# junshutang/Make-It-3D

Hardware: AMD Instinct MI355X
Metric: SDS train-steps/sec (NeRF render+SD U-Net fwd+bwd) @128x128 (higher is better)
Workload: dtype f32 hash grid (fp32 gather, fp32 gradient contributions accumulated in 64-bit fixed point) + f16 MFMA MLP (torch.autocast semantics; the planes between gather, MLP and scatter hold the binary16 values autocast rounds them to), f16 U-Net

## Files before the change

### include/mi3d.h

```cpp
#ifndef MI3D_H
#define MI3D_H

#include <stddef.h>
#include <stdint.h>

#ifdef __cplusplus
extern "C" {
#endif

#define MI3D_MAX_LEVELS 16
#define MI3D_MAX_POINTS 16

int mi3d_abi_version(void);
const char *mi3d_last_error_string(int err);


int mi3d_near_far_from_aabb(const float *rays_o, const float *rays_d, const float *aabb, uint32_t N,
                            float min_near, float *nears, float *fars, void *stream);
int mi3d_sph_from_ray(const float *rays_o, const float *rays_d, float radius, uint32_t N, float *coords,
                      void *stream);
int mi3d_morton3D(const int32_t *coords, uint32_t N, int32_t *indices, void *stream);
int mi3d_morton3D_invert(const int32_t *indices, uint32_t N, int32_t *coords, void *stream);
int mi3d_packbits(const float *grid, uint32_t N, float density_thresh, uint8_t *bitfield, void *stream);

int mi3d_march_rays_train(const float *rays_o, const float *rays_d, const uint8_t *grid, float bound,
                          float dt_gamma, uint32_t max_steps, uint32_t N, uint32_t C, uint32_t H, uint32_t M,
                          const float *nears, const float *fars, float *xyzs, float *dirs, float *deltas,
                          int32_t *rays, int32_t *counter, const float *noises, void *stream);
int mi3d_march_zero_tail(const int32_t *counter, uint32_t align, uint32_t M, float *xyzs, float *dirs,
                         float *deltas, void *stream);

int mi3d_composite_rays_train_forward(const float *sigmas, const float *rgbs, const float *deltas,
                                      const int32_t *rays, uint32_t M, uint32_t N, float T_thresh,
                                      float *weights_sum, float *depth, float *image, void *stream);
int mi3d_composite_rays_train_backward(const float *grad_weights_sum, const float *grad_image,
                                       const float *sigmas, const float *rgbs, const float *deltas,
                                       const int32_t *rays, const float *weights_sum, const float *image,
                                       uint32_t M, uint32_t N, float T_thresh, float *grad_sigmas,
                                       float *grad_rgbs, void *stream);
int mi3d_composite_rays_train_backward_depth(const float *grad_weights_sum, const float *grad_depth,
                                             const float *grad_image, const float *sigmas, const float *rgbs,
                                             const float *deltas, const int32_t *rays, const float *weights_sum,
                                             const float *depth, const float *image, uint32_t M, uint32_t N,
                                             float T_thresh, float *grad_sigmas, float *grad_rgbs, void *stream);
int mi3d_composite_sdf_rays_train_forward(const float *sigmas, const float *rgbs, const float *deltas,
                                          const int32_t *rays, uint32_t M, uint32_t N, float T_thresh,
                                          float *weights_sum, float *depth, float *image, void *stream);
int mi3d_composite_sdf_rays_train_backward(const float *grad_weights_sum, const float *grad_image,
                                           const float *sigmas, const float *rgbs, const float *deltas,
                                           const int32_t *rays, const float *weights_sum, const float *image,
                                           uint32_t M, uint32_t N, float T_thresh, float *grad_sigmas,
                                           float *grad_rgbs, void *stream);

int mi3d_march_rays(uint32_t n_alive, uint32_t n_step, const int32_t *rays_alive, const float *rays_t,
                    const float *rays_o, const float *rays_d, float bound, float dt_gamma, uint32_t max_steps,
                    uint32_t C, uint32_t H, const uint8_t *grid, const float *nears, const float *fars,
                    float *xyzs, float *dirs, float *deltas, const float *noises, void *stream);
int mi3d_composite_rays(uint32_t n_alive, uint32_t n_step, float T_thresh, int32_t *rays_alive, float *rays_t,
                        const float *sigmas, const float *rgbs, const float *normals, const float *deltas,
                        float *weights_sum, float *depth, float *image, float *normal, void *stream);
int mi3d_composite_sdf_rays(uint32_t n_alive, uint32_t n_step, float T_thresh, int32_t *rays_alive,
                            float *rays_t, const float *sigmas, const float *rgbs, const float *deltas,
                            float *weights_sum, float *depth, float *image, void *stream);

int mi3d_infer_begin(int32_t *ctl, int32_t *rays_alive, uint32_t N, uint32_t align, void *stream);
int mi3d_march_rays_ctl(const int32_t *ctl, uint32_t n_alive_max, const int32_t *rays_alive, const float *rays_t,
                        const float *rays_o, const float *rays_d, float bound, float dt_gamma, uint32_t max_steps,
                        uint32_t C, uint32_t H, const uint8_t *grid, const float *fars, float *xyzs, float *dirs,
                        float *deltas, const float *noises, void *stream);
int mi3d_composite_rays_ctl(const int32_t *ctl, uint32_t n_alive_max, float T_thresh, int32_t *rays_alive,
                            float *rays_t, const float *sigmas, const float *rgbs, const float *normals,
                            const float *deltas, float *weights_sum, float *depth, float *image, float *normal,
                            void *stream);
int mi3d_compact_alive_ctl(int32_t *ctl, const int32_t *rays_alive_in, int32_t *rays_alive_out, uint32_t N,
                           uint32_t align, uint32_t max_steps, void *stream);

int mi3d_infer_begin2(int32_t *ctl, int32_t *rays_alive, uint32_t N, uint32_t budget_rows, uint32_t step_min,
                      uint32_t step_max, void *stream);
int mi3d_march_rays_compact_ctl(int32_t *ctl, uint32_t n_alive_max, const int32_t *rays_alive, const float *rays_t,
                                const float *rays_o, const float *rays_d, float bound, float dt_gamma, uint32_t max_steps,
                                uint32_t C, uint32_t H, const uint8_t *grid, const float *fars, uint32_t rows_cap,
                                float *xyzs, float *dirs, float *deltas, int32_t *ray_slab, float *t_next,
                                const float *noises, void *stream);
int mi3d_composite_rays_compact_ctl(const int32_t *ctl, uint32_t n_alive_max, float T_thresh, int32_t *rays_alive,
                                    float *rays_t, const int32_t *ray_slab, const float *t_next, const float *sigmas,
                                    const float *rgbs, const float *normals, const float *deltas, float *weights_sum,
                                    float *depth, float *image, float *normal, void *stream);
int mi3d_compact_alive_ctl2(int32_t *ctl, const int32_t *rays_alive_in, int32_t *rays_alive_out, uint32_t N,
                            uint32_t max_steps, void *stream);


uint32_t mi3d_hashgrid_levels(uint32_t n_levels, uint32_t base_resolution, float per_level_scale,
                              uint32_t log2_hashmap_size, uint32_t *offsets_host, uint32_t *resolutions_host,
                              float *scales_host);

int mi3d_hashgrid_forward(const float *x, uint32_t n, const float *params, uint32_t n_levels,
                          uint32_t base_resolution, float per_level_scale, uint32_t log2_hashmap_size,
                          float *out, void *stream);
int mi3d_hashgrid_backward(const float *x, uint32_t n, const float *dout, uint32_t n_levels,
                           uint32_t base_resolution, float per_level_scale, uint32_t log2_hashmap_size,
                           float *grad_params, void *stream);


int mi3d_grid_encode_points(const float *x, const float *x2, uint32_t n, const int32_t *count,
                            const float *offsets_host, uint32_t P0, uint32_t P, float bound, const float *params,
                            uint32_t n_levels, uint32_t base_resolution, float per_level_scale,
                            uint32_t log2_hashmap_size, float *out, void *stream);
int mi3d_grid_encode_points_planes(const float *x, const float *x2, uint32_t n, const float *offsets_host, uint32_t P0,
                                   uint32_t P, float bound, const float *params, uint32_t n_levels,
                                   uint32_t base_resolution, float per_level_scale, uint32_t log2_hashmap_size, float step,
                                   void *out_planes, int out_half, void *stream);
int mi3d_grid_encode_points_planes_counted(const float *x, const float *x2, uint32_t n, const int32_t *count,
                                           const float *offsets_host, uint32_t P0, uint32_t P, float bound,
                                           const float *params, uint32_t n_levels, uint32_t base_resolution,
                                           float per_level_scale, uint32_t log2_hashmap_size, float step, void *out_planes,
                                           int out_half, void *stream);
int mi3d_grid_scatter_points(const float *x, const float *x2, uint32_t n, const int32_t *count,
                             const float *offsets_host, uint32_t P0, uint32_t P, float bound, const float *dout,
                             uint32_t n_levels, uint32_t base_resolution, float per_level_scale,
                             uint32_t log2_hashmap_size, float step, float *grad_params, void *stream);

size_t mi3d_grid_scatter_binned_workspace(uint32_t n, uint32_t P, float bound, float step, uint32_t n_levels,
                                          uint32_t base_resolution, float per_level_scale, uint32_t log2_hashmap_size);
int mi3d_grid_scatter_binned(const float *x, const float *x2, uint32_t n, const float *offsets_host, uint32_t P0,
                             uint32_t P, float bound, const void *dout_planes, int dout_half, uint32_t n_levels,
                             uint32_t base_resolution, float per_level_scale, uint32_t log2_hashmap_size, float step,
                             void *workspace, size_t workspace_bytes, float *grad_params, void *stream);
int mi3d_grid_scatter_binned_plus(const float *x, const float *x2, uint32_t n, const float *offsets_host, uint32_t P0,
                                  uint32_t P, float bound, const void *dout_planes, const void *extra_point0_planes,
                                  int dout_half, uint32_t n_levels, uint32_t base_resolution, float per_level_scale,
                                  uint32_t log2_hashmap_size, float step, void *workspace, size_t workspace_bytes,
                                  float *grad_params, void *stream);

int mi3d_grid_encode_plan(uint32_t n, float bound, float step, uint32_t n_levels, uint32_t base_resolution,
                          float per_level_scale, uint32_t log2_hashmap_size, uint32_t *n_segments, uint32_t *segments);
int mi3d_grid_scatter_plan(uint32_t n, uint32_t P, float bound, float step, uint32_t n_levels, uint32_t base_resolution,
                           float per_level_scale, uint32_t log2_hashmap_size, size_t workspace_bytes,
                           unsigned long long *out);
int mi3d_grid_level_routes(uint32_t n_levels, uint32_t base_resolution, float per_level_scale, uint32_t log2_hashmap_size,
                           int stencil_points, int32_t *kinds);


int mi3d_mlp_supported(uint32_t dim_in, uint32_t dim_hidden, uint32_t dim_out, uint32_t num_layers);
int mi3d_mlp_forward(const void *x, uint32_t x_plane_rows, int planes_half, uint32_t n, const float *W1,
                     const float *b1, const float *W2, const float *b2,
                     const float *W3, const float *b3, uint32_t dim_in, uint32_t dim_hidden, uint32_t dim_out,
                     int half_mode, float *out, void *stream);
int mi3d_mlp_forward_counted(const void *x, uint32_t x_plane_rows, int planes_half, uint32_t n, const int32_t *count,
                             uint32_t n_stride, const float *W1, const float *b1, const float *W2, const float *b2,
                             const float *W3, const float *b3, uint32_t dim_in, uint32_t dim_hidden, uint32_t dim_out,
                             int half_mode, float *out, void *stream);
int mi3d_mlp_backward(const void *x, uint32_t x_plane_rows, int planes_half, const float *dout, uint32_t n,
                      const float *W1, const float *b1, const float *W2, const float *b2, const float *W3,
                      const float *b3, uint32_t dim_in, uint32_t dim_hidden, uint32_t dim_out, int half_mode, void *dx,
                      uint32_t dx_plane_rows, float *dW1, float *db1, float *dW2, float *db2, float *dW3, float *db3,
                      void *stream);


int mi3d_field_head_forward(const float *h, const float *x, const float *x2, uint32_t n, const float *offsets_host,
                            uint32_t P, float bound, float blob_density, float blob_radius, float epsilon, float *sigma,
                            float *albedo, float *normal, float *normal2, void *stream);
int mi3d_field_head_forward_counted(const float *h, const float *x, const float *x2, uint32_t n, const int32_t *count,
                                    const float *offsets_host, uint32_t P, float bound, float blob_density,
                                    float blob_radius, float epsilon, float *sigma, float *albedo, float *normal,
                                    float *normal2, void *stream);
int mi3d_field_head_backward(const float *h, const float *x, const float *x2, uint32_t n, const float *offsets_host,
                             uint32_t P, uint32_t P_active, float bound, float blob_density, float blob_radius,
                             float epsilon, const float *dsigma, const float *dalbedo, const float *dnormal,
                             const float *dnormal2, float *dh, void *stream);


int mi3d_sumsq_accumulate(const float *x, size_t n, float *acc, void *stream);
int mi3d_adan_step(float *param, float *grad, float *exp_avg, float *exp_avg_sq, float *exp_avg_diff,
                   float *neg_pre_grad, size_t count, const float *grad_sumsq, float max_grad_norm, float clip_eps,
                   int first_step, float beta1, float beta2, float beta3, float bias_correction1,
                   float bias_correction2, float bias_correction3_sqrt, float lr, float weight_decay, float eps,
                   int no_prox, void *stream);


size_t mi3d_points_rasterize_workspace(uint32_t P, uint32_t H, uint32_t W, float radius);
int mi3d_points_rasterize(const float *points_ndc, uint32_t P, uint32_t H, uint32_t W, float radius,
                          uint32_t points_per_pixel, void *workspace, size_t workspace_bytes, int32_t *idx, float *zbuf,
                          float *dists, void *stream);
int mi3d_points_composite_forward(const int32_t *idx, const float *dists, uint32_t H, uint32_t W, uint32_t points_per_pixel,
                                  const float *features, uint32_t C, double radius, float *out, void *stream);
int mi3d_points_composite_backward(const int32_t *idx, const float *dists, uint32_t H, uint32_t W,
                                   uint32_t points_per_pixel, const float *grad_out, uint32_t C, double radius,
                                   float *grad_features, void *stream);


size_t mi3d_mc_workspace(uint32_t Rx, uint32_t Ry, uint32_t Rz);
int mi3d_mc_case(uint32_t case_index, int8_t *edges_host);
int mi3d_mc_count(const float *vol, uint32_t Rx, uint32_t Ry, uint32_t Rz, float iso, void *ws, size_t ws_bytes,
                  unsigned long long *counts, void *stream);
int mi3d_mc_scan(uint32_t Rx, uint32_t Ry, uint32_t Rz, void *ws, size_t ws_bytes, unsigned long long *counts,
                 void *stream);
int mi3d_mc_emit(const float *vol, uint32_t Rx, uint32_t Ry, uint32_t Rz, float iso, const float *origin_host,
                 const float *spacing_host, void *ws, size_t ws_bytes, unsigned long long *counts, float *vertices,
                 unsigned long long nv_cap, int32_t *triangles, unsigned long long nt_cap, void *stream);


uint32_t mi3d_atlas_cell(unsigned long long nt, uint32_t T);
int mi3d_atlas_uv(unsigned long long nt, uint32_t T, float *vt, void *stream);
int mi3d_atlas_positions(const float *vertices, unsigned long long nv, const int32_t *triangles, unsigned long long nt,
                         uint32_t T, uint32_t ssaa, uint32_t row0, uint32_t rows, float *xyz, int32_t *owner,
                         unsigned long long *bad, void *stream);
int mi3d_texture_pack(const float *albedo, const int32_t *owner, uint32_t T, uint32_t ssaa, uint32_t rows, uint8_t *image,
                      void *stream);


uint32_t mi3d_groupnorm_chunks(uint32_t HW);
int mi3d_groupnorm_stats(const void *x, uint32_t B, uint32_t C, uint32_t HW, uint32_t G, float *ws, void *stream);
int mi3d_groupnorm_act_forward(const void *x, const float *ws, const float *weight, const float *bias, uint32_t B,
                               uint32_t C, uint32_t HW, uint32_t G, float eps, int act, void *y, float *mean, float *rstd,
                               void *stream);
int mi3d_groupnorm_act_backward_sums(const void *x, const void *dy, const float *mean, const float *rstd,
                                     const float *weight, const float *bias, uint32_t B, uint32_t C, uint32_t HW,
                                     uint32_t G, int act, float *partial, void *stream);
int mi3d_groupnorm_act_backward(const void *x, const void *dy, const float *mean, const float *rstd, const float *weight,
                                const float *bias, const float *partial, uint32_t B, uint32_t C, uint32_t HW, uint32_t G,
                                int act, void *dx, void *stream);


int mi3d_canny_classify(const uint8_t *image, uint32_t H, uint32_t W, int32_t low, int32_t high, uint8_t *cls,
                        unsigned long long *counts, void *stream);
int mi3d_canny_hysteresis(uint8_t *cls, uint32_t H, uint32_t W, uint32_t sweeps, int32_t *changed, void *stream);


size_t mi3d_pc_unproject_workspace(uint32_t H, uint32_t W);
int mi3d_pc_unproject(const double *depth, const uint8_t *mask, uint32_t H, uint32_t W, const double *kinv_host,
                      const double *c2w_host, void *ws, size_t ws_bytes, double *points, unsigned long long cap,
                      unsigned long long *count, void *stream);
int mi3d_pc_project(const double *points, unsigned long long n, const double *rt_host, const double *k_host, double *xy,
                    double *z, void *stream);
int mi3d_pc_zmin(const double *points, unsigned long long n, const double *rt_host, const double *k_host, uint32_t H,
                 uint32_t W, unsigned long long *zkeys, void *stream);
int mi3d_pc_visible(const double *points, unsigned long long n, const double *rt_host, const double *k_host, uint32_t H,
                    uint32_t W, const unsigned long long *zkeys, uint8_t *visible, void *stream);
int mi3d_box_morph(const float *src, float *dst, uint32_t H, uint32_t W, uint32_t kh, uint32_t kw, int dilate,
                   void *stream);
int mi3d_pc_cano_filter(const double *points, unsigned long long n, const double *rt_host, const double *k_host,
                        const float *cano_depth, uint32_t H, uint32_t W, uint8_t *keep, void *stream);
int mi3d_pc_colour(const double *points, unsigned long long n, const double *rt_host, const double *k_host,
                   const float *image, uint32_t H, uint32_t W, float *colour, void *stream);

#ifdef __cplusplus
}
#endif
#endif
```

### make-it-3d_amd/csrc/field.hip

```cpp
#include <hip/hip_runtime.h>

#include "../../include/mi3d.h"
#include "mi3d_dev.h"
#include "lds_transpose.h"

#ifndef MI3D_MLP_LDS_TRANSPOSE
#define MI3D_MLP_LDS_TRANSPOSE 1
#endif

namespace {

constexpr int kWave = 64;
constexpr int kWavesPerWG = 4;
constexpr int DIN = 32, HID = 64, DOUT = 4;
constexpr int NTH = HID / 32;

using f32x16 = __attribute__((ext_vector_type(16))) float;
using f32x4 = __attribute__((ext_vector_type(4))) float;
using f32x2 = __attribute__((ext_vector_type(2))) float;
using half8 = __attribute__((ext_vector_type(8))) _Float16;
using half2v = __attribute__((ext_vector_type(2))) _Float16;
using ushort8v = __attribute__((ext_vector_type(8))) unsigned short;

inline hipStream_t as_stream(void *s) { return reinterpret_cast<hipStream_t>(s); }

__device__ __forceinline__ int rowmap(int q, int h) { return (q & 3) + 8 * (q >> 2) + 4 * h; }

struct F16 {
    using elem = _Float16;
    static constexpr int kUnits = 2;
    static constexpr bool kLdsTranspose = MI3D_MLP_LDS_TRANSPOSE != 0;
    struct KB { half8 v[2]; };
    __device__ static __forceinline__ float round(float x) { return (float)(_Float16)x; }
    __device__ static __forceinline__ void set(KB &k, int q, float x) { k.v[q >> 3][q & 7] = (_Float16)x; }
    __device__ static __forceinline__ void set_pair_bits(KB &k, int j, uint32_t bits) {
        const half2v hv = __builtin_bit_cast(half2v, bits);
        k.v[j >> 2][2 * (j & 3)] = hv[0];
        k.v[j >> 2][2 * (j & 3) + 1] = hv[1];
    }
    __device__ static __forceinline__ void mma(f32x16 &acc, const KB &a, const KB &b) {
        acc = __builtin_amdgcn_mfma_f32_32x32x16_f16(a.v[0], b.v[0], acc, 0, 0, 0);
        acc = __builtin_amdgcn_mfma_f32_32x32x16_f16(a.v[1], b.v[1], acc, 0, 0, 0);
    }
    [[maybe_unused]] static constexpr int kSteps = 2;
    __device__ static __forceinline__ void mma_step(f32x16 &acc, const KB &a, const KB &b, int s) {
        acc = __builtin_amdgcn_mfma_f32_32x32x16_f16(a.v[s], b.v[s], acc, 0, 0, 0);
    }
    __device__ static __forceinline__ void mma_lo(f32x16 &acc, const KB &a, const KB &b) {
        acc = __builtin_amdgcn_mfma_f32_32x32x16_f16(a.v[0], b.v[0], acc, 0, 0, 0);
    }
    __device__ static __forceinline__ KB load_block(const char *blk, int lane) {
        KB k;
        k.v[0] = *reinterpret_cast<const half8 *>(blk + (0 * kWave + lane) * 16);
        k.v[1] = *reinterpret_cast<const half8 *>(blk + (1 * kWave + lane) * 16);
        return k;
    }
    __device__ static __forceinline__ KB relu(const f32x16 &acc) {
        KB k;
#pragma unroll
        for (int j = 0; j < 8; ++j) {
            const f32x2 pr = {acc[2 * j], acc[2 * j + 1]};
            half2v hv = __builtin_convertvector(pr, half2v);
            hv = __builtin_elementwise_maximum(hv, half2v{(_Float16)0, (_Float16)0});
            k.v[j >> 2][2 * (j & 3)] = hv[0];
            k.v[j >> 2][2 * (j & 3) + 1] = hv[1];
        }
        return k;
    }
    __device__ static __forceinline__ KB masked(const f32x16 &d, const KB &act) {
        KB k;
        const unsigned ones = 0x00010001u;
        using u32x4 = __attribute__((ext_vector_type(4))) uint32_t;
#pragma unroll
        for (int u = 0; u < 2; ++u) {
            const u32x4 aw = __builtin_bit_cast(u32x4, act.v[u]);
            u32x4 o;
#pragma unroll
            for (int j = 0; j < 4; ++j) {
                const f32x2 pr = {d[8 * u + 2 * j], d[8 * u + 2 * j + 1]};
                const unsigned dv = __builtin_bit_cast(unsigned, __builtin_convertvector(pr, half2v));
                unsigned m = aw[j];
                asm("v_pk_min_u16 %0, %1, %2\n\tv_pk_mul_lo_u16 %0, %0, %3"
                    : "=&v"(m) : "v"(m), "s"(ones), "v"(dv));
                o[j] = m;
            }
            k.v[u] = __builtin_bit_cast(half8, o);
        }
        return k;
    }
    __device__ static __forceinline__ KB cast(const f32x16 &acc) {
        KB k;
#pragma unroll
        for (int j = 0; j < 8; ++j) {
            const f32x2 pr = {acc[2 * j], acc[2 * j + 1]};
            const half2v hv = __builtin_convertvector(pr, half2v);
            k.v[j >> 2][2 * (j & 3)] = hv[0];
            k.v[j >> 2][2 * (j & 3) + 1] = hv[1];
        }
        return k;
    }
    __device__ static __forceinline__ float sum(const KB &k) {
        float s = 0.f;
        const half2v ones = {(_Float16)1, (_Float16)1};
        using u32x4 = __attribute__((ext_vector_type(4))) uint32_t;
#pragma unroll
        for (int u = 0; u < 2; ++u) {
            const u32x4 w = __builtin_bit_cast(u32x4, k.v[u]);
#pragma unroll
            for (int j = 0; j < 4; ++j) {
                const uint32_t wj = w[j];
                s = __builtin_amdgcn_fdot2(__builtin_bit_cast(half2v, wj), ones, s, false);
            }
        }
        return s;
    }
};

struct F32 {
    using elem = float;
    static constexpr int kUnits = 4;
    static constexpr bool kLdsTranspose = false;
    struct KB { float v[16]; };
    __device__ static __forceinline__ float round(float x) { return x; }
    __device__ static __forceinline__ void set(KB &k, int q, float x) { k.v[q] = x; }
    __device__ static __forceinline__ void set_pair_bits(KB &k, int j, uint32_t bits) {
        const half2v hv = __builtin_bit_cast(half2v, bits);
        k.v[2 * j] = (float)hv[0];
        k.v[2 * j + 1] = (float)hv[1];
    }
    __device__ static __forceinline__ void mma(f32x16 &acc, const KB &a, const KB &b) {
#pragma unroll
        for (int q = 0; q < 16; ++q) acc = __builtin_amdgcn_mfma_f32_32x32x2f32(a.v[q], b.v[q], acc, 0, 0, 0);
    }
    static constexpr int kSteps = 16;
    __device__ static __forceinline__ void mma_step(f32x16 &acc, const KB &a, const KB &b, int s) {
        acc = __builtin_amdgcn_mfma_f32_32x32x2f32(a.v[s], b.v[s], acc, 0, 0, 0);
    }
    __device__ static __forceinline__ void mma_lo(f32x16 &acc, const KB &a, const KB &b) {
#pragma unroll
        for (int q = 0; q < 8; ++q) acc = __builtin_amdgcn_mfma_f32_32x32x2f32(a.v[q], b.v[q], acc, 0, 0, 0);
    }
    __device__ static __forceinline__ KB load_block(const char *blk, int lane) {
        KB k;
#pragma unroll
        for (int u = 0; u < 4; ++u) {
            const f32x4 t = *reinterpret_cast<const f32x4 *>(blk + (u * kWave + lane) * 16);
            k.v[4 * u] = t[0]; k.v[4 * u + 1] = t[1]; k.v[4 * u + 2] = t[2]; k.v[4 * u + 3] = t[3];
        }
        return k;
    }
    __device__ static __forceinline__ KB relu(const f32x16 &acc) {
        KB k;
#pragma unroll
        for (int q = 0; q < 16; ++q) k.v[q] = fmaxf(acc[q], 0.f);
        return k;
    }
    __device__ static __forceinline__ KB masked(const f32x16 &d, const KB &act) {
        KB k;
#pragma unroll
        for (int q = 0; q < 16; ++q) k.v[q] = act.v[q] > 0.f ? d[q] : 0.f;
        return k;
    }
    __device__ static __forceinline__ KB cast(const f32x16 &acc) {
        KB k;
#pragma unroll
        for (int q = 0; q < 16; ++q) k.v[q] = acc[q];
        return k;
    }
    __device__ static __forceinline__ float sum(const KB &k) {
        float s = 0.f;
#pragma unroll
        for (int q = 0; q < 16; ++q) s += k.v[q];
        return s;
    }
};

template <class P> constexpr int block_bytes() { return P::kUnits * kWave * 16; }

enum : int {
    B_W1 = 0,
    B_W2 = B_W1 + NTH,
    B_W3 = B_W2 + NTH * NTH,
    B_W3T = B_W3 + NTH,
    B_W2T = B_W3T + NTH,
    B_W1T = B_W2T + NTH * NTH,
    B_ID = B_W1T + NTH,
    B_ALL_COUNT = B_ID + 1,
};

struct Weights {
    const float *W1, *b1, *W2, *b2, *W3, *b3;
};

template <class P>
__device__ void build_blocks(char *lds, float *bias , const Weights &w, int n_blocks) {
    using T = typename P::elem;
    for (int e = threadIdx.x; e < n_blocks * kWave * 16; e += blockDim.x) {
        const int blk = e / (kWave * 16), r = e % (kWave * 16), lane = r / 16, q = r % 16;
        const int nl = lane & 31, h = lane >> 5;
        const int kd = rowmap(q, h), kx = 16 * h + q;
        float v = 0.f;
        if (blk < B_W2) {
            const int tn = blk - B_W1;
            v = w.W1[(32 * tn + nl) * DIN + kx];
        } else if (blk < B_W3) {
            const int tn = (blk - B_W2) / NTH, tk = (blk - B_W2) % NTH;
            v = w.W2[(32 * tn + nl) * HID + 32 * tk + kd];
        } else if (blk < B_W3T) {
            const int tk = blk - B_W3;
            v = nl < DOUT ? w.W3[nl * HID + 32 * tk + kd] : 0.f;
        } else if (blk < B_W2T) {
            const int tn = blk - B_W3T;
            v = kx < DOUT ? w.W3[kx * HID + 32 * tn + nl] : 0.f;
        } else if (blk < B_W1T) {
            const int tn = (blk - B_W2T) / NTH, tk = (blk - B_W2T) % NTH;
            v = w.W2[(32 * tk + kd) * HID + 32 * tn + nl];
        } else if (blk < B_ID) {
            const int tk = blk - B_W1T;
            v = w.W1[(32 * tk + kd) * DIN + nl];
        } else {
            v = nl == kx ? 1.f : 0.f;
        }
        constexpr int per_unit = 16 / (int)sizeof(T);
        T *dst = reinterpret_cast<T *>(lds + (size_t)blk * block_bytes<P>() + ((q / per_unit) * kWave + lane) * 16);
        dst[q % per_unit] = (T)v;
    }
    for (int e = threadIdx.x; e < HID + HID + 32; e += blockDim.x) {
        float v = 0.f;
        if (e < HID) v = w.b1[e];
        else if (e < 2 * HID) v = w.b2[e - HID];
        else if (e - 2 * HID < DOUT) v = w.b3[e - 2 * HID];
        bias[e] = P::round(v);
    }
}

__device__ __forceinline__ void load_rows_raw(const float *__restrict__ x, size_t row, size_t n, int h,
                                              size_t plane_rows, float (&raw)[16], int planes_half = 0) {
    row = row < n ? row : n - 1;
    if (plane_rows != 0 && planes_half) {
#pragma unroll
        for (int j = 0; j < 8; ++j) {
            const uint32_t u = reinterpret_cast<const uint32_t *>(x)[(size_t)(8 * h + j) * plane_rows + row];
            raw[2 * j] = (float)__builtin_bit_cast(_Float16, (unsigned short)(u & 0xFFFFu));
            raw[2 * j + 1] = (float)__builtin_bit_cast(_Float16, (unsigned short)(u >> 16));
        }
    } else if (plane_rows == 0) {
        const f32x4 *src = reinterpret_cast<const f32x4 *>(x + row * DIN + 16 * h);
#pragma unroll
        for (int c = 0; c < 4; ++c) {
            const f32x4 t = src[c];
#pragma unroll
            for (int i = 0; i < 4; ++i) raw[4 * c + i] = t[i];
        }
    } else {
#pragma unroll
        for (int j = 0; j < 8; ++j) {
            const f32x2 t = *reinterpret_cast<const f32x2 *>(x + ((size_t)(8 * h + j) * plane_rows + row) * 2);
            raw[2 * j] = t[0];
            raw[2 * j + 1] = t[1];
        }
    }
}
template <class P> __device__ __forceinline__ typename P::KB rows_kb(const float (&raw)[16]) {
    typename P::KB k;
#pragma unroll
    for (int q = 0; q < 16; ++q) P::set(k, q, raw[q]);
    return k;
}
[[maybe_unused]] __device__ __forceinline__ void load_rows_half(const float *__restrict__ x, size_t row, size_t n, int h,
                                               size_t plane_rows, uint32_t (&u)[8]) {
    row = row < n ? row : n - 1;
#pragma unroll
    for (int j = 0; j < 8; ++j) u[j] = reinterpret_cast<const uint32_t *>(x)[(size_t)(8 * h + j) * plane_rows + row];
}
template <class P> __device__ __forceinline__ typename P::KB rows_kb_half(const uint32_t (&u)[8]) {
    typename P::KB k;
#pragma unroll
    for (int j = 0; j < 8; ++j) P::set_pair_bits(k, j, u[j]);
    return k;
}

__device__ __forceinline__ f32x4 load_dout_raw(const float *__restrict__ dout, size_t row, size_t n) {
    return *reinterpret_cast<const f32x4 *>(dout + (row < n ? row : n - 1) * DOUT);
}
template <class P> __device__ __forceinline__ typename P::KB dout_kb(const f32x4 &t, bool keep) {
    typename P::KB k;
#pragma unroll
    for (int q = 0; q < 16; ++q) P::set(k, q, (q < 4 && keep) ? t[q] : 0.f);
    return k;
}

__device__ __forceinline__ f32x16 splat(float v) {
    f32x16 a;
#pragma unroll
    for (int q = 0; q < 16; ++q) a[q] = v;
    return a;
}
__device__ __forceinline__ f32x16 bias_rows(const float *bias, int h) {
    f32x16 a;
#pragma unroll
    for (int q = 0; q < 16; ++q) a[q] = bias[rowmap(q, h)];
    return a;
}
struct Grads {
    float *dW1, *db1, *dW2, *db2, *dW3, *db3;
};

template <class P, int U, int WPS, bool HP>
__global__ __launch_bounds__(kWave *kWavesPerWG, WPS) void k_mlp_backward(const float *x, uint32_t x_planes,
                                                                           int , const float *__restrict__ dout,
                                                                           uint32_t n, Weights w, float *dx,
                                                                           uint32_t dx_planes, Grads g) {
    extern __shared__ __attribute__((aligned(16))) char lds[];
    float *bias = reinterpret_cast<float *>(lds + (size_t)B_ALL_COUNT * block_bytes<P>());
    build_blocks<P>(lds, bias, w, B_ALL_COUNT);
    __syncthreads();
    const int lane = threadIdx.x & (kWave - 1), p = lane & 31, h = lane >> 5;
    const uint32_t wave = blockIdx.x * kWavesPerWG + threadIdx.x / kWave, n_waves = gridDim.x * kWavesPerWG;
    const uint32_t n_tiles = (n + 31) / 32;
    using KB = typename P::KB;
    auto blk = [&](int b) {
        int l = lane;
        asm volatile("" : "+v"(l));
        return P::load_block(lds + (size_t)b * block_bytes<P>(), l);
    };

    f32x16 gW2[NTH][NTH], gW1[NTH], gW3[NTH];
    float gb1[NTH], gb2[NTH], gb3 = 0.f;
#pragma unroll
    for (int a = 0; a < NTH; ++a) {
        gW1[a] = splat(0.f); gW3[a] = splat(0.f); gb1[a] = 0.f; gb2[a] = 0.f;
#pragma unroll
        for (int b = 0; b < NTH; ++b) gW2[a][b] = splat(0.f);
    }

    float raw[HP ? 1 : U][16];
    uint32_t rawh[HP ? U : 1][8];
    f32x4 dor[U];
#pragma unroll
    for (int u = 0; u < U; ++u) {
        const size_t r0 = ((size_t)wave + (size_t)u * n_waves) * 32 + p;
        if constexpr (HP) load_rows_half(x, r0, n, h, x_planes, rawh[u]);
        else load_rows_raw(x, r0, n, h, x_planes, raw[u]);
        dor[u] = load_dout_raw(dout, r0, n);
    }
    for (uint32_t tile = wave; tile < n_tiles; tile += U * n_waves) {
        size_t row[U];
        bool valid[U];
        KB X[U], dO[U];
#pragma unroll
        for (int u = 0; u < U; ++u) {
            row[u] = ((size_t)tile + (size_t)u * n_waves) * 32 + p;
            valid[u] = row[u] < n;
            if constexpr (HP) X[u] = rows_kb_half<P>(rawh[u]);
            else X[u] = rows_kb<P>(raw[u]);
            dO[u] = dout_kb<P>(dor[u], valid[u] && h == 0);
        }
        if (tile + U * n_waves < n_tiles) {
#pragma unroll
            for (int u = 0; u < U; ++u) {
                const size_t rn = ((size_t)tile + (size_t)(U + u) * n_waves) * 32 + p;
                if constexpr (HP) load_rows_half(x, rn, n, h, x_planes, rawh[u]);
                else load_rows_raw(x, rn, n, h, x_planes, raw[u]);
                dor[u] = load_dout_raw(dout, rn, n);
            }
        }

        KB H1[U][NTH], H2[U][NTH], dH2[U][NTH], dH1[U][NTH];
        {
            f32x16 acc[U][NTH];
#pragma unroll
            for (int t = 0; t < NTH; ++t)
#pragma unroll
                for (int u = 0; u < U; ++u) acc[u][t] = bias_rows(bias + 32 * t, h);
            {
                KB Wb[NTH];
#pragma unroll
                for (int t = 0; t < NTH; ++t) Wb[t] = blk(B_W1 + t);
#pragma unroll
                for (int st = 0; st < P::kSteps; ++st)
#pragma unroll
                    for (int t = 0; t < NTH; ++t)
#pragma unroll
                        for (int u = 0; u < U; ++u) P::mma_step(acc[u][t], Wb[t], X[u], st);
            }
#pragma unroll
            for (int t = 0; t < NTH; ++t)
#pragma unroll
                for (int u = 0; u < U; ++u) H1[u][t] = P::relu(acc[u][t]);
        }
        {
            f32x16 acc[U][NTH];
#pragma unroll
            for (int t = 0; t < NTH; ++t)
#pragma unroll
                for (int u = 0; u < U; ++u) acc[u][t] = bias_rows(bias + HID + 32 * t, h);
#pragma unroll
            for (int tk = 0; tk < NTH; ++tk) {
                KB Wb[NTH];
#pragma unroll
                for (int t = 0; t < NTH; ++t) Wb[t] = blk(B_W2 + t * NTH + tk);
#pragma unroll
                for (int st = 0; st < P::kSteps; ++st)
#pragma unroll
                    for (int t = 0; t < NTH; ++t)
#pragma unroll
                        for (int u = 0; u < U; ++u) P::mma_step(acc[u][t], Wb[t], H1[u][tk], st);
            }
#pragma unroll
            for (int t = 0; t < NTH; ++t)
#pragma unroll
                for (int u = 0; u < U; ++u) H2[u][t] = P::relu(acc[u][t]);
        }
        {
            f32x16 acc[U][NTH];
            KB Wb[NTH];
#pragma unroll
            for (int t = 0; t < NTH; ++t) Wb[t] = blk(B_W3T + t);
#pragma unroll
            for (int t = 0; t < NTH; ++t)
#pragma unroll
                for (int u = 0; u < U; ++u) { acc[u][t] = splat(0.f); P::mma_lo(acc[u][t], Wb[t], dO[u]); }
#pragma unroll
            for (int t = 0; t < NTH; ++t)
#pragma unroll
                for (int u = 0; u < U; ++u) dH2[u][t] = P::masked(acc[u][t], H2[u][t]);
        }
        {
            f32x16 acc[U][NTH];
#pragma unroll
            for (int t = 0; t < NTH; ++t)
#pragma unroll
                for (int u = 0; u < U; ++u) acc[u][t] = splat(0.f);
#pragma unroll
            for (int tk = 0; tk < NTH; ++tk) {
                KB Wb[NTH];
#pragma unroll
                for (int t = 0; t < NTH; ++t) Wb[t] = blk(B_W2T + t * NTH + tk);
#pragma unroll
                for (int st = 0; st < P::kSteps; ++st)
#pragma unroll
                    for (int t = 0; t < NTH; ++t)
#pragma unroll
                        for (int u = 0; u < U; ++u) P::mma_step(acc[u][t], Wb[t], dH2[u][tk], st);
            }
#pragma unroll
            for (int t = 0; t < NTH; ++t)
#pragma unroll
                for (int u = 0; u < U; ++u) dH1[u][t] = P::masked(acc[u][t], H1[u][t]);
        }
        {
            f32x16 acc[U];
#pragma unroll
            for (int u = 0; u < U; ++u) acc[u] = splat(0.f);
#pragma unroll
            for (int tk = 0; tk < NTH; ++tk) {
                const KB Wb = blk(B_W1T + tk);
#pragma unroll
                for (int st = 0; st < P::kSteps; ++st)
#pragma unroll
                    for (int u = 0; u < U; ++u) P::mma_step(acc[u], Wb, dH1[u][tk], st);
            }
#pragma unroll
            for (int u = 0; u < U; ++u) {
                if (valid[u] && !dx_planes) {
                    float *dst = dx + row[u] * DIN + 4 * h;
#pragma unroll
                    for (int c = 0; c < 4; ++c) {
                        f32x4 o = {acc[u][4 * c], acc[u][4 * c + 1], acc[u][4 * c + 2], acc[u][4 * c + 3]};
                        __builtin_nontemporal_store(o, reinterpret_cast<f32x4 *>(dst + 8 * c));
                    }
                } else if (valid[u] && HP) {
#pragma unroll
                    for (int c = 0; c < 4; ++c) {
                        const size_t lvl = 4 * c + 2 * h;
                        const half2v a = __builtin_convertvector((f32x2){acc[u][4 * c], acc[u][4 * c + 1]}, half2v);
                        const half2v b = __builtin_convertvector((f32x2){acc[u][4 * c + 2], acc[u][4 * c + 3]}, half2v);
                        reinterpret_cast<uint32_t *>(dx)[lvl * dx_planes + row[u]] = __builtin_bit_cast(uint32_t, a);
                        reinterpret_cast<uint32_t *>(dx)[(lvl + 1) * dx_planes + row[u]] = __builtin_bit_cast(uint32_t, b);
                    }
                } else if (valid[u]) {
#pragma unroll
                    for (int c = 0; c < 4; ++c) {
                        f32x2 a = {acc[u][4 * c], acc[u][4 * c + 1]}, b = {acc[u][4 * c + 2], acc[u][4 * c + 3]};
                        const size_t lvl = 4 * c + 2 * h;
                        __builtin_nontemporal_store(a, reinterpret_cast<f32x2 *>(dx + (lvl * dx_planes + row[u]) * 2));
                        __builtin_nontemporal_store(b, reinterpret_cast<f32x2 *>(dx + ((lvl + 1) * dx_planes + row[u]) * 2));
                    }
                }
            }
        }

        KB H1p[U][NTH];
        {
            f32x16 acc[U][NTH];
#pragma unroll
            for (int t = 0; t < NTH; ++t)
#pragma unroll
                for (int u = 0; u < U; ++u) acc[u][t] = splat(bias[32 * t + p]);
            KB Wb[NTH];
#pragma unroll
            for (int t = 0; t < NTH; ++t) Wb[t] = blk(B_W1 + t);
#pragma unroll
            for (int st = 0; st < P::kSteps; ++st)
#pragma unroll
                for (int t = 0; t < NTH; ++t)
#pragma unroll
                    for (int u = 0; u < U; ++u) P::mma_step(acc[u][t], X[u], Wb[t], st);
#pragma unroll
            for (int t = 0; t < NTH; ++t)
#pragma unroll
                for (int u = 0; u < U; ++u) H1p[u][t] = P::relu(acc[u][t]);
        }
        KB dH2p[U][NTH];
        {
            KB H2p[U][NTH], dOp[U];
            {
                f32x16 acc[U][NTH];
#pragma unroll
                for (int t = 0; t < NTH; ++t)
#pragma unroll
                    for (int u = 0; u < U; ++u) acc[u][t] = splat(bias[HID + 32 * t + p]);
#pragma unroll
                for (int tk = 0; tk < NTH; ++tk) {
                    KB Wb[NTH];
#pragma unroll
                    for (int t = 0; t < NTH; ++t) Wb[t] = blk(B_W2 + t * NTH + tk);
#pragma unroll
                    for (int st = 0; st < P::kSteps; ++st)
#pragma unroll
                        for (int t = 0; t < NTH; ++t)
#pragma unroll
                            for (int u = 0; u < U; ++u) P::mma_step(acc[u][t], H1[u][tk], Wb[t], st);
                }
#pragma unroll
                for (int t = 0; t < NTH; ++t)
#pragma unroll
                    for (int u = 0; u < U; ++u) H2p[u][t] = P::relu(acc[u][t]);
            }
            {
                const KB Id = blk(B_ID);
                f32x16 tO[U];
#pragma unroll
                for (int u = 0; u < U; ++u) { tO[u] = splat(0.f); P::mma_lo(tO[u], dO[u], Id); }
#pragma unroll
                for (int u = 0; u < U; ++u) { dOp[u] = P::cast(tO[u]); gb3 += P::sum(dOp[u]); }
            }
#pragma unroll
            for (int u = 0; u < U; ++u)
#pragma unroll
                for (int st = 0; st < P::kSteps; ++st)
#pragma unroll
                    for (int t = 0; t < NTH; ++t) P::mma_step(gW3[t], dOp[u], H2p[u][t], st);
            {
                f32x16 d[U][NTH];
                KB Wb[NTH];
#pragma unroll
                for (int t = 0; t < NTH; ++t) Wb[t] = blk(B_W3T + t);
#pragma unroll
                for (int t = 0; t < NTH; ++t)
#pragma unroll
                    for (int u = 0; u < U; ++u) { d[u][t] = splat(0.f); P::mma_lo(d[u][t], dO[u], Wb[t]); }
#pragma unroll
                for (int t = 0; t < NTH; ++t)
#pragma unroll
                    for (int u = 0; u < U; ++u) {
                        dH2p[u][t] = P::masked(d[u][t], H2p[u][t]);
                        gb2[t] += P::sum(dH2p[u][t]);
                    }
            }
        }
#pragma unroll
        for (int u = 0; u < U; ++u)
#pragma unroll
            for (int st = 0; st < P::kSteps; ++st)
#pragma unroll
                for (int ti = 0; ti < NTH; ++ti)
#pragma unroll
                    for (int tj = 0; tj < NTH; ++tj) P::mma_step(gW2[ti][tj], dH2p[u][ti], H1p[u][tj], st);
        {
            KB dH1p[U][NTH], Xp[U];
            {
                f32x16 d[U][NTH];
#pragma unroll
                for (int t = 0; t < NTH; ++t)
#pragma unroll
                    for (int u = 0; u < U; ++u) d[u][t] = splat(0.f);
#pragma unroll
                for (int tk = 0; tk < NTH; ++tk) {
                    KB Wb[NTH];
#pragma unroll
                    for (int t = 0; t < NTH; ++t) Wb[t] = blk(B_W2T + t * NTH + tk);
#pragma unroll
                    for (int st = 0; st < P::kSteps; ++st)
#pragma unroll
                        for (int t = 0; t < NTH; ++t)
#pragma unroll
                            for (int u = 0; u < U; ++u) P::mma_step(d[u][t], dH2[u][tk], Wb[t], st);
                }
#pragma unroll
                for (int t = 0; t < NTH; ++t)
#pragma unroll
                    for (int u = 0; u < U; ++u) {
                        dH1p[u][t] = P::masked(d[u][t], H1p[u][t]);
                        gb1[t] += P::sum(dH1p[u][t]);
                    }
            }
            {
                const KB Id = blk(B_ID);
                f32x16 tX[U];
#pragma unroll
                for (int u = 0; u < U; ++u) tX[u] = splat(0.f);
#pragma unroll
                for (int st = 0; st < P::kSteps; ++st)
#pragma unroll
                    for (int u = 0; u < U; ++u) P::mma_step(tX[u], X[u], Id, st);
#pragma unroll
                for (int u = 0; u < U; ++u) Xp[u] = P::cast(tX[u]);
            }
#pragma unroll
            for (int u = 0; u < U; ++u)
#pragma unroll
                for (int st = 0; st < P::kSteps; ++st)
#pragma unroll
                    for (int t = 0; t < NTH; ++t) P::mma_step(gW1[t], dH1p[u][t], Xp[u], st);
        }
    }

    __syncthreads();
    float *red = reinterpret_cast<float *>(lds);
    constexpr int OFF_W1 = 0, OFF_B1 = OFF_W1 + HID * DIN, OFF_W2 = OFF_B1 + HID, OFF_B2 = OFF_W2 + HID * HID,
                  OFF_W3 = OFF_B2 + HID, OFF_B3 = OFF_W3 + DOUT * HID, TOTAL = OFF_B3 + DOUT;
    for (int e = threadIdx.x; e < TOTAL; e += blockDim.x) red[e] = 0.f;
    __syncthreads();
#pragma unroll
    for (int q = 0; q < 16; ++q) {
        const int r = rowmap(q, h);
#pragma unroll
        for (int ti = 0; ti < NTH; ++ti) {
            atomicAdd(&red[OFF_W1 + (32 * ti + r) * DIN + p], gW1[ti][q]);
#pragma unroll
            for (int tj = 0; tj < NTH; ++tj) atomicAdd(&red[OFF_W2 + (32 * ti + r) * HID + 32 * tj + p], gW2[ti][tj][q]);
            if (r < DOUT) atomicAdd(&red[OFF_W3 + r * HID + 32 * ti + p], gW3[ti][q]);
        }
    }
#pragma unroll
    for (int t = 0; t < NTH; ++t) {
        atomicAdd(&red[OFF_B1 + 32 * t + p], gb1[t]);
        atomicAdd(&red[OFF_B2 + 32 * t + p], gb2[t]);
    }
    if (p < DOUT) atomicAdd(&red[OFF_B3 + p], gb3);
    __syncthreads();
    for (int e = threadIdx.x; e < TOTAL; e += blockDim.x) {
        const float v = red[e];
        float *dst = e < OFF_B1 ? g.dW1 + (e - OFF_W1)
                   : e < OFF_W2 ? g.db1 + (e - OFF_B1)
                   : e < OFF_B2 ? g.dW2 + (e - OFF_W2)
                   : e < OFF_W3 ? g.db2 + (e - OFF_B2)
                   : e < OFF_B3 ? g.dW3 + (e - OFF_W3)
                                : g.db3 + (e - OFF_B3);
        if (v != 0.f) unsafeAtomicAdd(dst, v);
    }
}

template <int NTH, int LAYERS> struct Blk {
    static constexpr int W1 = 0;
    static constexpr int W2 = W1 + NTH;
    static constexpr int W3 = W2 + (LAYERS == 3 ? NTH * NTH : 0);
    static constexpr int FWD_COUNT = W3 + NTH;
    static constexpr int W3T = FWD_COUNT;
    static constexpr int W2T = W3T + NTH;
    static constexpr int W1T = W2T + (LAYERS == 3 ? NTH * NTH : 0);
    static constexpr int IDX = W1T + NTH;
    static constexpr int IDD = IDX + 1;
    static constexpr int ALL_COUNT = IDD + 1;
    static constexpr int BIAS_TILES = 2 * NTH + 1;
};

template <class P, int NTH, int LAYERS>
__device__ void build_blocks_g(char *lds, float *biasT, const Weights &w, int din, int n_blocks) {
    using T = typename P::elem;
    using B = Blk<NTH, LAYERS>;
    constexpr int H = 32 * NTH;
    for (int e = threadIdx.x; e < n_blocks * kWave * 16; e += blockDim.x) {
        const int blk = e / (kWave * 16), r = e % (kWave * 16), lane = r / 16, q = r % 16;
        const int nl = lane & 31, h = lane >> 5;
        const int kd = rowmap(q, h), kx = 16 * h + q;
        float v = 0.f;
        if (blk < B::W2) {
            const int tn = blk - B::W1;
            v = kx < din ? w.W1[(32 * tn + nl) * din + kx] : 0.f;
        } else if (blk < B::W3) {
            const int tn = (blk - B::W2) / NTH, tk = (blk - B::W2) % NTH;
            v = w.W2[(32 * tn + nl) * H + 32 * tk + kd];
        } else if (blk < B::W3T) {
            const int tk = blk - B::W3;
            v = nl < DOUT ? w.W3[nl * H + 32 * tk + kd] : 0.f;
        } else if (blk < B::W2T) {
            const int tn = blk - B::W3T;
            v = kx < DOUT ? w.W3[kx * H + 32 * tn + nl] : 0.f;
        } else if (blk < B::W1T) {
            const int tn = (blk - B::W2T) / NTH, tk = (blk - B::W2T) % NTH;
            v = w.W2[(32 * tk + kd) * H + 32 * tn + nl];
        } else if (blk < B::IDX) {
            const int tk = blk - B::W1T;
            v = nl < din ? w.W1[(32 * tk + kd) * din + nl] : 0.f;
        } else if (blk == B::IDX) {
            v = nl == kx ? 1.f : 0.f;
        } else {
            v = nl == kd ? 1.f : 0.f;
        }
        constexpr int per_unit = 16 / (int)sizeof(T);
        T *dst = reinterpret_cast<T *>(lds + (size_t)blk * block_bytes<P>() + ((q / per_unit) * kWave + lane) * 16);
        dst[q % per_unit] = (T)v;
    }
    for (int e = threadIdx.x; e < B::BIAS_TILES * 32; e += blockDim.x) {
        const int tile = e / 32, h = (e % 32) / 16, q = e % 16, row = rowmap(q, h);
        float v = 0.f;
        if (tile < NTH) v = w.b1[32 * tile + row];
        else if (tile < 2 * NTH) v = LAYERS == 3 ? w.b2[32 * (tile - NTH) + row] : 0.f;
        else v = row < DOUT ? w.b3[row] : 0.f;
        biasT[e] = P::round(v);
    }
}
__device__ __forceinline__ f32x16 bias_tile(const float *biasT, int tile, int h) {
    const f32x4 *src = reinterpret_cast<const f32x4 *>(biasT + (tile * 2 + h) * 16);
    f32x16 a;
#pragma unroll
    for (int c = 0; c < 4; ++c) {
        const f32x4 t = src[c];
        a[4 * c] = t[0]; a[4 * c + 1] = t[1]; a[4 * c + 2] = t[2]; a[4 * c + 3] = t[3];
    }
    return a;
}

template <bool FULL = false>
__device__ __forceinline__ void load_rows_half_g(const float *__restrict__ x, size_t row, size_t n, int h,
                                                 size_t plane_rows, uint32_t last_plane, uint32_t (&u)[8]) {
    row = row < n ? row : n - 1;
    if constexpr (FULL) {
        const uint32_t *src = reinterpret_cast<const uint32_t *>(x) + ((size_t)(8 * h) * plane_rows + row);
#pragma unroll
        for (int j = 0; j < 8; ++j) u[j] = src[(size_t)j * plane_rows];
        return;
    }
#pragma unroll
    for (int j = 0; j < 8; ++j) {
        const uint32_t pl = (uint32_t)(8 * h + j) < last_plane ? (uint32_t)(8 * h + j) : last_plane;
        u[j] = reinterpret_cast<const uint32_t *>(x)[(size_t)pl * plane_rows + row];
    }
}
__device__ __forceinline__ void load_rows_raw_g(const float *__restrict__ x, size_t row, size_t n, int h,
                                                size_t plane_rows, uint32_t din, float (&raw)[16]) {
    row = row < n ? row : n - 1;
    const uint32_t last_plane = din / 2 - 1;
    if (plane_rows == 0 && din == DIN) {
        const f32x4 *src = reinterpret_cast<const f32x4 *>(x + row * DIN + 16 * h);
#pragma unroll
        for (int c = 0; c < 4; ++c) {
            const f32x4 t = src[c];
#pragma unroll
            for (int i = 0; i < 4; ++i) raw[4 * c + i] = t[i];
        }
    } else if (plane_rows == 0) {
#pragma unroll
        for (int q = 0; q < 16; ++q) {
            const uint32_t f = (uint32_t)(16 * h + q) < din ? (uint32_t)(16 * h + q) : din - 1;
            raw[q] = x[row * din + f];
        }
    } else {
#pragma unroll
        for (int j = 0; j < 8; ++j) {
            const uint32_t pl = (uint32_t)(8 * h + j) < last_plane ? (uint32_t)(8 * h + j) : last_plane;
            const f32x2 t = *reinterpret_cast<const f32x2 *>(x + ((size_t)pl * plane_rows + row) * 2);
            raw[2 * j] = t[0];
            raw[2 * j + 1] = t[1];
        }
    }
}

template <class P, int NTH, int LAYERS, bool HP>
__global__ __launch_bounds__(kWave *kWavesPerWG, 2) void k_mlp_fwd_g(const float *__restrict__ x, uint32_t x_planes,
                                                                        uint32_t n, uint32_t din, Weights w,
                                                                        float *__restrict__ out,
                                                                        const int32_t *__restrict__ count, uint32_t n_stride) {
    using B = Blk<NTH, LAYERS>;
    using KB = typename P::KB;
    extern __shared__ __attribute__((aligned(16))) char lds[];
    float *biasT = reinterpret_cast<float *>(lds + (size_t)B::FWD_COUNT * block_bytes<P>());
    build_blocks_g<P, NTH, LAYERS>(lds, biasT, w, (int)din, B::FWD_COUNT);
    __syncthreads();
    const int lane = threadIdx.x & (kWave - 1), p = lane & 31, h = lane >> 5;
    const uint32_t wave = blockIdx.x * kWavesPerWG + threadIdx.x / kWave, n_waves = gridDim.x * kWavesPerWG;
    const uint32_t n_tiles = (n + 31) / 32;
    auto blk = [&](int b) {
        int l = lane;
        asm volatile("" : "+v"(l));
        return P::load_block(lds + (size_t)b * block_bytes<P>(), l);
    };
    auto bias = [&](int tile) {
        int hh = h;
        asm volatile("" : "+v"(hh));
        return bias_tile(biasT, tile, hh);
    };
    const uint32_t last_plane = din / 2 - 1;
    const uint32_t c_rows = count ? (uint32_t)max(*count, 0) : 0xFFFFFFFFu;
    for (uint32_t tile = wave; tile < n_tiles; tile += n_waves) {
        bool live = true;
        if (count) {
            const uint32_t s0 = (tile * 32u) % n_stride;
            if (s0 >= c_rows && s0 + 32u <= n_stride) continue;
            live = (s0 + (uint32_t)p) % n_stride < c_rows;
        }
        const size_t row = (size_t)tile * 32 + p;
        KB X;
        if constexpr (HP) {
            uint32_t u[8];
            load_rows_half_g(x, row, n, h, x_planes, last_plane, u);
            X = rows_kb_half<P>(u);
        } else {
            float raw[16];
            load_rows_raw_g(x, row, n, h, x_planes, din, raw);
            X = rows_kb<P>(raw);
        }
        KB H1[NTH], HL[NTH];
#pragma unroll
        for (int t = 0; t < NTH; ++t) {
            f32x16 acc = bias(t);
            P::mma(acc, blk(B::W1 + t), X);
            H1[t] = P::relu(acc);
        }
        if constexpr (LAYERS == 3) {
#pragma unroll
            for (int t = 0; t < NTH; ++t) {
                f32x16 acc = bias(NTH + t);
#pragma unroll
                for (int tk = 0; tk < NTH; ++tk) P::mma(acc, blk(B::W2 + t * NTH + tk), H1[tk]);
                HL[t] = P::relu(acc);
            }
        } else {
#pragma unroll
            for (int t = 0; t < NTH; ++t) HL[t] = H1[t];
        }
        f32x16 acc = bias(2 * NTH);
#pragma unroll
        for (int tk = 0; tk < NTH; ++tk) P::mma(acc, blk(B::W3 + tk), HL[tk]);
        if (row < n && h == 0 && live) {
            f32x4 o = {P::round(acc[0]), P::round(acc[1]), P::round(acc[2]), P::round(acc[3])};
            __builtin_nontemporal_store(o, reinterpret_cast<f32x4 *>(out + row * DOUT));
        }
    }
}

template <class P, int NTH, int LAYERS, bool HP, bool FULL>
__global__ __launch_bounds__(kWave *kWavesPerWG, 2) void k_mlp_bwd_g(const float *x, uint32_t x_planes,
                                                                        const float *__restrict__ dout, uint32_t n,
                                                                        uint32_t din, Weights w, float *dx,
                                                                        uint32_t dx_planes, Grads g) {
    using B = Blk<NTH, LAYERS>;
    using KB = typename P::KB;
    constexpr int H = 32 * NTH;
    extern __shared__ __attribute__((aligned(16))) char lds[];
    float *biasT = reinterpret_cast<float *>(lds + (size_t)B::ALL_COUNT * block_bytes<P>());
    build_blocks_g<P, NTH, LAYERS>(lds, biasT, w, (int)din, B::ALL_COUNT);
    __syncthreads();
    const int lane = threadIdx.x & (kWave - 1), p = lane & 31, h = lane >> 5;
    const uint32_t wave = blockIdx.x * kWavesPerWG + threadIdx.x / kWave, n_waves = gridDim.x * kWavesPerWG;
    const uint32_t n_tiles = (n + 31) / 32;
    int lt = lane, ht = h;
    auto blk = [&](int b) { return P::load_block(lds + (size_t)b * block_bytes<P>(), lt); };
    auto blk_fresh = [&](int b) {
        int l = lane;
        asm volatile("" : "+v"(l));
        return P::load_block(lds + (size_t)b * block_bytes<P>(), l);
    };
    auto bias = [&](int tile) { return bias_tile(biasT, tile, ht); };
    [[maybe_unused]] mi3d_tr::lds_ptr tr_wr_d = nullptr, tr_wr_x = nullptr, tr_rd = nullptr;
    if constexpr (P::kLdsTranspose) {
        mi3d_tr::lds_ptr tile = mi3d_tr::to_lds(biasT + B::BIAS_TILES * 32) + (threadIdx.x / kWave) * mi3d_tr::kTileBytes;
        tr_wr_d = tile + mi3d_tr::write_offset_d(lane);
        tr_wr_x = tile + mi3d_tr::write_offset_x(lane);
        tr_rd = tile + mi3d_tr::read_offset(lane);
    }
    auto transpose = [&](const KB &a, int id_block) {
        if constexpr (P::kLdsTranspose) {
            KB r;
            if (id_block == B::IDX) mi3d_tr::write_tile<true>(tr_wr_x, a.v[0], a.v[1]);
            else mi3d_tr::write_tile<false>(tr_wr_d, a.v[0], a.v[1]);
            mi3d_tr::read_tile(tr_rd, r.v[0], r.v[1]);
            return r;
        } else {
            f32x16 t = splat(0.f);
            P::mma(t, a, blk_fresh(id_block));
            return P::cast(t);
        }
    };
    const uint32_t last_plane = FULL ? (uint32_t)(DIN / 2 - 1) : din / 2 - 1;

    f32x16 gW1[NTH], gW2[NTH][NTH], gW3[NTH];
    float gb1[NTH], gb2[NTH], gb3 = 0.f;
#pragma unroll
    for (int a = 0; a < NTH; ++a) {
        gW1[a] = splat(0.f); gW3[a] = splat(0.f); gb1[a] = 0.f; gb2[a] = 0.f;
#pragma unroll
        for (int b = 0; b < NTH; ++b) gW2[a][b] = splat(0.f);
    }

    float raw[HP ? 1 : 16];
    uint32_t rawh[HP ? 8 : 1];
    f32x4 dor;
    {
        const size_t r0 = (size_t)wave * 32 + p;
        if constexpr (HP) load_rows_half_g<FULL && P::kLdsTranspose>(x, r0, n, h, x_planes, last_plane, rawh);
        else load_rows_raw_g(x, r0, n, h, x_planes, din, raw);
        dor = load_dout_raw(dout, r0, n);
    }
    for (uint32_t tile = wave; tile < n_tiles; tile += n_waves) {
        const size_t row = (size_t)tile * 32 + p;
        const bool valid = row < n;
        uint32_t xp = x_planes, dxp = dx_planes;
        asm volatile("" : "+s"(xp), "+s"(dxp), "+v"(lt), "+v"(ht));
        KB X;
        if constexpr (HP) X = rows_kb_half<P>(rawh);
        else X = rows_kb<P>(raw);
        const KB dO = dout_kb<P>(dor, valid && h == 0);
        auto prefetch = [&]() {
            if (tile + n_waves < n_tiles) {
                const size_t rn = ((size_t)tile + n_waves) * 32 + p;
                if constexpr (HP) load_rows_half_g<FULL && P::kLdsTranspose>(x, rn, n, P::kLdsTranspose ? ht : h, xp, last_plane, rawh);
                else load_rows_raw_g(x, rn, n, P::kLdsTranspose ? ht : h, xp, din, raw);
                dor = load_dout_raw(dout, rn, n);
            }
        };
        constexpr bool late_prefetch = P::kLdsTranspose && HP;
        if constexpr (!late_prefetch) prefetch();
        KB H1p[NTH], HL[NTH];
        {
            KB H1[NTH];
#pragma unroll
            for (int t = 0; t < NTH; ++t) {
                f32x16 acc = bias(t);
                P::mma(acc, blk(B::W1 + t), X);
                H1[t] = P::relu(acc);
            }
            if constexpr (LAYERS == 3) {
#pragma unroll
                for (int t = 0; t < NTH; ++t) {
                    f32x16 acc = bias(NTH + t);
#pragma unroll
                    for (int tk = 0; tk < NTH; ++tk) P::mma(acc, blk(B::W2 + t * NTH + tk), H1[tk]);
                    HL[t] = P::relu(acc);
                }
            } else {
#pragma unroll
                for (int t = 0; t < NTH; ++t) HL[t] = H1[t];
            }
#pragma unroll
            for (int t = 0; t < NTH; ++t) H1p[t] = transpose(H1[t], B::IDD);
        }
        KB dHL[NTH];
#pragma unroll
        for (int t = 0; t < NTH; ++t) {
            f32x16 acc = splat(0.f);
            P::mma_lo(acc, blk(B::W3T + t), dO);
            dHL[t] = P::masked(acc, HL[t]);
        }
        {
            KB dOp;
            if constexpr (P::kLdsTranspose) {
                dOp = transpose(dO, B::IDX);
            } else {
                f32x16 tO = splat(0.f);
                P::mma_lo(tO, dO, blk_fresh(B::IDX));
                dOp = P::cast(tO);
            }
            gb3 += P::sum(dOp);
#pragma unroll
            for (int t = 0; t < NTH; ++t) {
                const KB HLp = LAYERS == 3 ? transpose(HL[t], B::IDD) : H1p[t];
                P::mma(gW3[t], dOp, HLp);
            }
        }
        KB dH1p[NTH];
        if constexpr (LAYERS == 3) {
#pragma unroll
            for (int ti = 0; ti < NTH; ++ti) {
                const KB dHLp = transpose(dHL[ti], B::IDD);
                gb2[ti] += P::sum(dHLp);
#pragma unroll
                for (int tj = 0; tj < NTH; ++tj) P::mma(gW2[ti][tj], dHLp, H1p[tj]);
            }
#pragma unroll
            for (int t = 0; t < NTH; ++t) {
                f32x16 acc = splat(0.f);
#pragma unroll
                for (int tk = 0; tk < NTH; ++tk) P::mma(acc, dHL[tk], blk(B::W2T + t * NTH + tk));
                dH1p[t] = P::masked(acc, H1p[t]);
            }
        } else {
#pragma unroll
            for (int t = 0; t < NTH; ++t) dH1p[t] = transpose(dHL[t], B::IDD);
        }
        {
            const KB Xp = transpose(X, B::IDX);
            if constexpr (late_prefetch) prefetch();
#pragma unroll
            for (int t = 0; t < NTH; ++t) {
                gb1[t] += P::sum(dH1p[t]);
                P::mma(gW1[t], dH1p[t], Xp);
            }
        }
        {
            f32x16 acc = splat(0.f);
#pragma unroll
            for (int tk = 0; tk < NTH; ++tk) {
                const KB dH1 = LAYERS == 3 ? transpose(dH1p[tk], B::IDD) : dHL[tk];
                P::mma(acc, blk(B::W1T + tk), dH1);
            }
            const bool full = FULL || din == (uint32_t)DIN;
            if constexpr (HP) {
            if (valid) {
                uint32_t *dxh = reinterpret_cast<uint32_t *>(dx) + row;
                uint32_t pk[8];
#pragma unroll
                for (int c = 0; c < 4; ++c) {
                    pk[2 * c] = __builtin_bit_cast(uint32_t, __builtin_convertvector((f32x2){acc[4 * c], acc[4 * c + 1]}, half2v));
                    pk[2 * c + 1] = __builtin_bit_cast(uint32_t, __builtin_convertvector((f32x2){acc[4 * c + 2], acc[4 * c + 3]}, half2v));
                }
                if (FULL && P::kLdsTranspose) {
                    uint32_t *dst = dxh + (size_t)(2 * h) * dxp;
#pragma unroll
                    for (int c = 0; c < 4; ++c) {
                        dst[(size_t)(4 * c) * dxp] = pk[2 * c];
                        dst[(size_t)(4 * c + 1) * dxp] = pk[2 * c + 1];
                    }
                } else if (full) {
#pragma unroll
                    for (int c = 0; c < 4; ++c) {
                        dxh[(size_t)(4 * c + 2 * h) * dxp] = pk[2 * c];
                        dxh[(size_t)(4 * c + 2 * h + 1) * dxp] = pk[2 * c + 1];
                    }
                } else {
#pragma unroll
                    for (int c = 0; c < 4; ++c) {
                        const uint32_t lvl = 4 * c + 2 * h;
                        if (lvl <= last_plane) dxh[(size_t)lvl * dxp] = pk[2 * c];
                        if (lvl + 1 <= last_plane) dxh[(size_t)(lvl + 1) * dxp] = pk[2 * c + 1];
                    }
                }
            }
            } else {
            if (valid && !dxp) {
                if (full) {
                    float *dst = dx + row * DIN + 4 * h;
#pragma unroll
                    for (int c = 0; c < 4; ++c) {
                        f32x4 o = {acc[4 * c], acc[4 * c + 1], acc[4 * c + 2], acc[4 * c + 3]};
                        __builtin_nontemporal_store(o, reinterpret_cast<f32x4 *>(dst + 8 * c));
                    }
                } else {
#pragma unroll
                    for (int q = 0; q < 16; ++q)
                        if ((uint32_t)rowmap(q, h) < din) dx[row * din + rowmap(q, h)] = acc[q];
                }
            } else if (valid) {
#pragma unroll
                for (int c = 0; c < 4; ++c) {
                    f32x2 a = {acc[4 * c], acc[4 * c + 1]}, b = {acc[4 * c + 2], acc[4 * c + 3]};
                    const uint32_t lvl = 4 * c + 2 * h;
                    if (lvl <= last_plane)
                        __builtin_nontemporal_store(a, reinterpret_cast<f32x2 *>(dx + ((size_t)lvl * dxp + row) * 2));
                    if (lvl + 1 <= last_plane)
                        __builtin_nontemporal_store(b, reinterpret_cast<f32x2 *>(dx + ((size_t)(lvl + 1) * dxp + row) * 2));
                }
            }
            }
        }
    }

    __syncthreads();
    float *red = reinterpret_cast<float *>(lds);
    const int OFF_W1 = 0, OFF_B1 = OFF_W1 + H * (int)din, OFF_W2 = OFF_B1 + H,
              OFF_B2 = OFF_W2 + (LAYERS == 3 ? H * H : 0), OFF_W3 = OFF_B2 + (LAYERS == 3 ? H : 0),
              OFF_B3 = OFF_W3 + DOUT * H, TOTAL = OFF_B3 + DOUT;
    for (int e = threadIdx.x; e < TOTAL; e += blockDim.x) red[e] = 0.f;
    __syncthreads();
#pragma unroll
    for (int q = 0; q < 16; ++q) {
        const int r = rowmap(q, h);
#pragma unroll
        for (int ti = 0; ti < NTH; ++ti) {
            if (p < (int)din) atomicAdd(&red[OFF_W1 + (32 * ti + r) * (int)din + p], gW1[ti][q]);
            if constexpr (LAYERS == 3) {
#pragma unroll
                for (int tj = 0; tj < NTH; ++tj) atomicAdd(&red[OFF_W2 + (32 * ti + r) * H + 32 * tj + p], gW2[ti][tj][q]);
            }
            if (r < DOUT) atomicAdd(&red[OFF_W3 + r * H + 32 * ti + p], gW3[ti][q]);
        }
    }
#pragma unroll
    for (int t = 0; t < NTH; ++t) {
        atomicAdd(&red[OFF_B1 + 32 * t + p], gb1[t]);
        if constexpr (LAYERS == 3) atomicAdd(&red[OFF_B2 + 32 * t + p], gb2[t]);
    }
    if (p < DOUT) atomicAdd(&red[OFF_B3 + p], gb3);
    __syncthreads();
    for (int e = threadIdx.x; e < TOTAL; e += blockDim.x) {
        const float v = red[e];
        float *dst = e < OFF_B1 ? g.dW1 + (e - OFF_W1)
                   : e < OFF_W2 ? g.db1 + (e - OFF_B1)
                   : e < OFF_B2 ? g.dW2 + (e - OFF_W2)
                   : e < OFF_W3 ? g.db2 + (e - OFF_B2)
                   : e < OFF_B3 ? g.dW3 + (e - OFF_W3)
                                : g.db3 + (e - OFF_B3);
        if (v != 0.f) unsafeAtomicAdd(dst, v);
    }
}

struct HeadArgs {
    const float *x, *x2;
    float offs[MI3D_MAX_POINTS * 3];
    uint32_t P;
    float bound, blob_density, two_r2, inv_2eps;
};

__device__ __forceinline__ float head_gauss(const HeadArgs &a, const float *base, uint32_t p) {
    float d2 = 0.f;
#pragma unroll
    for (int d = 0; d < 3; ++d) {
        const float v = fminf(a.bound, fmaxf(-a.bound, base[d] + a.offs[p * 3 + d]));
        d2 += v * v;
    }
    return a.blob_density * expf(-d2 / a.two_r2);
}

__device__ __forceinline__ void head_normal(const float s[6], float inv_2eps, float n[3], float v[3], float &c) {
    v[0] = -((s[0] - s[1]) * inv_2eps); v[1] = -((s[2] - s[3]) * inv_2eps); v[2] = -((s[4] - s[5]) * inv_2eps);
    const float ss = v[0] * v[0] + v[1] * v[1] + v[2] * v[2];
    c = fminf(1e32f, fmaxf(1e-20f, ss));
    const float r = 1.0f / sqrtf(c);
#pragma unroll
    for (int d = 0; d < 3; ++d) {
        float t = v[d] * r;
        if (t != t) t = 0.f;
        else if (t > 3.4028234663852886e38f) t = 3.4028234663852886e38f;
        else if (t < -3.4028234663852886e38f) t = -3.4028234663852886e38f;
        n[d] = t;
    }
}

__global__ void k_head_forward(const float4 *__restrict__ h, HeadArgs a, uint32_t n, float *__restrict__ sigma,
                               float *__restrict__ albedo, float *__restrict__ normal, float *__restrict__ normal2,
                               const int32_t *__restrict__ count) {
    const uint32_t s = blockIdx.x * blockDim.x + threadIdx.x;
    if (s >= n || (count && (int32_t)s >= *count)) return;
    float bx[3] = {a.x[(size_t)s * 3], a.x[(size_t)s * 3 + 1], a.x[(size_t)s * 3 + 2]};
    const float4 h0 = h[s];
    sigma[s] = expf(h0.x + head_gauss(a, bx, 0));
    albedo[(size_t)s * 3] = 1.0f / (1.0f + expf(-h0.y));
    albedo[(size_t)s * 3 + 1] = 1.0f / (1.0f + expf(-h0.z));
    albedo[(size_t)s * 3 + 2] = 1.0f / (1.0f + expf(-h0.w));
    float sg[6], nn[3], v[3], c;
#pragma unroll
    for (uint32_t p = 0; p < 6; ++p) sg[p] = expf(h[(size_t)(1 + p) * n + s].x + head_gauss(a, bx, 1 + p));
    head_normal(sg, a.inv_2eps, nn, v, c);
    normal[(size_t)s * 3] = nn[0]; normal[(size_t)s * 3 + 1] = nn[1]; normal[(size_t)s * 3 + 2] = nn[2];
    if (a.P == 13) {
        float b2[3] = {a.x2[(size_t)s * 3], a.x2[(size_t)s * 3 + 1], a.x2[(size_t)s * 3 + 2]};
#pragma unroll
        for (uint32_t p = 0; p < 6; ++p) sg[p] = expf(h[(size_t)(7 + p) * n + s].x + head_gauss(a, b2, 7 + p));
        head_normal(sg, a.inv_2eps, nn, v, c);
        normal2[(size_t)s * 3] = nn[0]; normal2[(size_t)s * 3 + 1] = nn[1]; normal2[(size_t)s * 3 + 2] = nn[2];
    }
}

__device__ __forceinline__ void head_normal_backward(const float u[6], float inv_2eps, const float dn_in[3], float du[6]) {
    float sg[6], nn[3], v[3], c;
#pragma unroll
    for (int p = 0; p < 6; ++p) sg[p] = expf(u[p]);
    head_normal(sg, inv_2eps, nn, v, c);
    const float ss = v[0] * v[0] + v[1] * v[1] + v[2] * v[2];
    const float r = 1.0f / sqrtf(c);
    float dn[3];
#pragma unroll
    for (int d = 0; d < 3; ++d) {
        const float t = v[d] * r;
        dn[d] = (t == t && fabsf(t) <= 3.4028234663852886e38f) ? dn_in[d] : 0.f;
    }
    const float dot = dn[0] * v[0] + dn[1] * v[1] + dn[2] * v[2];
    const bool inside = ss >= 1e-20f && ss <= 1e32f;
    const float k = inside ? dot * (r / c) : 0.f;
#pragma unroll
    for (int d = 0; d < 3; ++d) {
        const float dv = r * dn[d] - k * v[d];
        const float dg = -dv * inv_2eps;
        du[2 * d] = dg * expf(fminf(u[2 * d], 15.0f));
        du[2 * d + 1] = -dg * expf(fminf(u[2 * d + 1], 15.0f));
    }
}

__global__ void k_head_backward(const float4 *__restrict__ h, HeadArgs a, uint32_t n, uint32_t P_active,
                                const float *__restrict__ dsigma, const float *__restrict__ dalbedo,
                                const float *__restrict__ dnormal, const float *__restrict__ dnormal2,
                                float4 *__restrict__ dh) {
    const uint32_t s = blockIdx.x * blockDim.x + threadIdx.x;
    if (s >= n) return;
    float bx[3] = {a.x[(size_t)s * 3], a.x[(size_t)s * 3 + 1], a.x[(size_t)s * 3 + 2]};
    const float4 h0 = h[s];
    float4 g0;
    g0.x = (dsigma ? dsigma[s] : 0.f) * expf(fminf(h0.x + head_gauss(a, bx, 0), 15.0f));
    const float a0 = 1.0f / (1.0f + expf(-h0.y)), a1 = 1.0f / (1.0f + expf(-h0.z)), a2 = 1.0f / (1.0f + expf(-h0.w));
    g0.y = dalbedo ? dalbedo[(size_t)s * 3] * a0 * (1.0f - a0) : 0.f;
    g0.z = dalbedo ? dalbedo[(size_t)s * 3 + 1] * a1 * (1.0f - a1) : 0.f;
    g0.w = dalbedo ? dalbedo[(size_t)s * 3 + 2] * a2 * (1.0f - a2) : 0.f;
    dh[s] = g0;
    if (P_active < 7) return;
    float u[6], du[6], dn[3];
#pragma unroll
    for (uint32_t p = 0; p < 6; ++p) u[p] = h[(size_t)(1 + p) * n + s].x + head_gauss(a, bx, 1 + p);
#pragma unroll
    for (int d = 0; d < 3; ++d) dn[d] = dnormal ? dnormal[(size_t)s * 3 + d] : 0.f;
    head_normal_backward(u, a.inv_2eps, dn, du);
#pragma unroll
    for (uint32_t p = 0; p < 6; ++p) dh[(size_t)(1 + p) * n + s] = make_float4(du[p], 0.f, 0.f, 0.f);
    if (a.P == 13 && P_active == 13) {
        float b2[3] = {a.x2[(size_t)s * 3], a.x2[(size_t)s * 3 + 1], a.x2[(size_t)s * 3 + 2]};
#pragma unroll
        for (uint32_t p = 0; p < 6; ++p) u[p] = h[(size_t)(7 + p) * n + s].x + head_gauss(a, b2, 7 + p);
#pragma unroll
        for (int d = 0; d < 3; ++d) dn[d] = dnormal2 ? dnormal2[(size_t)s * 3 + d] : 0.f;
        head_normal_backward(u, a.inv_2eps, dn, du);
#pragma unroll
        for (uint32_t p = 0; p < 6; ++p) dh[(size_t)(7 + p) * n + s] = make_float4(du[p], 0.f, 0.f, 0.f);
    }
}

HeadArgs make_head_args(const float *x, const float *x2, const float *offsets_host, uint32_t P, float bound,
                        float blob_density, float blob_radius, float epsilon) {
    HeadArgs a;
    a.x = x; a.x2 = x2; a.P = P; a.bound = bound; a.blob_density = blob_density;
    a.two_r2 = (float)(2.0 * (double)blob_radius * (double)blob_radius);
    a.inv_2eps = 0.5f / epsilon;
    for (uint32_t i = 0; i < MI3D_MAX_POINTS * 3; ++i) a.offs[i] = i < P * 3 ? offsets_host[i] : 0.f;
    return a;
}

template <class P> constexpr size_t lds_bytes(int n_blocks) {
    return (size_t)n_blocks * block_bytes<P>() + (HID + HID + 32) * sizeof(float);
}
template <class P> constexpr size_t lds_bytes_g(int n_blocks, int bias_tiles, bool transposes = false) {
    return (size_t)n_blocks * block_bytes<P>() + (size_t)bias_tiles * 32 * sizeof(float) +
           (transposes && P::kLdsTranspose ? (size_t)kWavesPerWG * mi3d_tr::kTileBytes : 0u);
}

int grid_for(uint32_t n, int wgs_per_cu) {
    const uint32_t tiles = (n + 31) / 32, wgs = (tiles + kWavesPerWG - 1) / kWavesPerWG;
    const uint32_t cap = 256 * (uint32_t)wgs_per_cu;
    return (int)(wgs < cap ? (wgs ? wgs : 1) : cap);
}

bool dims_ok(uint32_t di, uint32_t dh, uint32_t dout, uint32_t layers) {
    return di >= 2 && di <= (uint32_t)DIN && di % 2 == 0 && (dh == 32 || dh == 64) && dout == DOUT &&
           (layers == 2 || layers == 3);
}

template <class P, int NTH, int LAYERS, bool HP>
void launch_fwd(dim3 grid, hipStream_t st, const float *x, uint32_t x_planes, uint32_t n, uint32_t din, const Weights &w,
                float *out, const int32_t *count, uint32_t n_stride) {
    using B = Blk<NTH, LAYERS>;
    hipLaunchKernelGGL((k_mlp_fwd_g<P, NTH, LAYERS, HP>), grid, dim3(kWave * kWavesPerWG),
                       lds_bytes_g<P>(B::FWD_COUNT, B::BIAS_TILES), st, x, x_planes, n, din, w, out, count, n_stride);
}
template <class P, int NTH, int LAYERS, bool HP>
void launch_bwd(dim3 grid, hipStream_t st, const float *x, uint32_t x_planes, const float *dout, uint32_t n, uint32_t din,
                const Weights &w, float *dx, uint32_t dx_planes, const Grads &g) {
    using B = Blk<NTH, LAYERS>;
    if (HP && P::kLdsTranspose && din == (uint32_t)DIN)
        hipLaunchKernelGGL((k_mlp_bwd_g<P, NTH, LAYERS, HP, HP && P::kLdsTranspose>), grid, dim3(kWave * kWavesPerWG),
                           lds_bytes_g<P>(B::ALL_COUNT, B::BIAS_TILES, true), st, x, x_planes, dout, n, din, w, dx, dx_planes, g);
    else
        hipLaunchKernelGGL((k_mlp_bwd_g<P, NTH, LAYERS, HP, false>), grid, dim3(kWave * kWavesPerWG),
                           lds_bytes_g<P>(B::ALL_COUNT, B::BIAS_TILES, true), st, x, x_planes, dout, n, din, w, dx, dx_planes, g);
}
#define MI3D_MLP_DISPATCH(FN, P, HP, nth, layers, ...)                     \
    do {                                                                   \
        if ((nth) == 2 && (layers) == 3) FN<P, 2, 3, HP>(__VA_ARGS__);     \
        else if ((nth) == 2) FN<P, 2, 2, HP>(__VA_ARGS__);                 \
        else if ((layers) == 3) FN<P, 1, 3, HP>(__VA_ARGS__);              \
        else FN<P, 1, 2, HP>(__VA_ARGS__);                                 \
    } while (0)

}

extern "C" {

int mi3d_mlp_supported(uint32_t dim_in, uint32_t dim_hidden, uint32_t dim_out, uint32_t num_layers) {
    return dims_ok(dim_in, dim_hidden, dim_out, num_layers) ? 1 : 0;
}

int mi3d_mlp_forward(const void *xv, uint32_t x_plane_rows, int planes_half, uint32_t n, const float *W1, const float *b1, const float *W2, const float *b2,
                     const float *W3, const float *b3, uint32_t dim_in, uint32_t dim_hidden, uint32_t dim_out,
                     int half_mode, float *out, void *stream) {
    return mi3d_mlp_forward_counted(xv, x_plane_rows, planes_half, n, nullptr, n ? n : 1u, W1, b1, W2, b2, W3, b3, dim_in,
                                    dim_hidden, dim_out, half_mode, out, stream);
}

int mi3d_mlp_forward_counted(const void *xv, uint32_t x_plane_rows, int planes_half, uint32_t n, const int32_t *count,
                             uint32_t n_stride, const float *W1, const float *b1, const float *W2, const float *b2,
                             const float *W3, const float *b3, uint32_t dim_in, uint32_t dim_hidden, uint32_t dim_out,
                             int half_mode, float *out, void *stream) {
    if (n_stride == 0) return (int)hipErrorInvalidValue;
    const uint32_t layers = (W2 == nullptr && b2 == nullptr) ? 2u : 3u;
    if (!dims_ok(dim_in, dim_hidden, dim_out, layers) || (x_plane_rows != 0 && x_plane_rows < n) ||
        (planes_half && (x_plane_rows == 0 || !half_mode)) || W1 == nullptr || b1 == nullptr || W3 == nullptr ||
        b3 == nullptr || (layers == 3 && (W2 == nullptr || b2 == nullptr)))
        return (int)hipErrorInvalidValue;
    if (n == 0) return 0;
    const float *x = reinterpret_cast<const float *>(xv);
    const Weights w{W1, b1, W2, b2, W3, b3};
    const int nth = (int)dim_hidden / 32;
    hipStream_t st = as_stream(stream);
    const dim3 grid(grid_for(n, MI3D_TUNE(MI3D_T_MLP_FWD_WGS_PER_CU, 5)));
    if (half_mode && planes_half) MI3D_MLP_DISPATCH(launch_fwd, F16, true, nth, layers, grid, st, x, x_plane_rows, n, dim_in, w, out, count, n_stride);
    else if (half_mode) MI3D_MLP_DISPATCH(launch_fwd, F16, false, nth, layers, grid, st, x, x_plane_rows, n, dim_in, w, out, count, n_stride);
    else MI3D_MLP_DISPATCH(launch_fwd, F32, false, nth, layers, grid, st, x, x_plane_rows, n, dim_in, w, out, count, n_stride);
    return (int)hipGetLastError();
}

int mi3d_mlp_backward(const void *xv, uint32_t x_plane_rows, int planes_half, const float *dout, uint32_t n, const float *W1, const float *b1,
                      const float *W2, const float *b2, const float *W3, const float *b3, uint32_t dim_in,
                      uint32_t dim_hidden, uint32_t dim_out, int half_mode, void *dxv, uint32_t dx_plane_rows, float *dW1, float *db1, float *dW2, float *db2, float *dW3, float *db3,
                      void *stream) {
    const uint32_t layers = (W2 == nullptr && b2 == nullptr) ? 2u : 3u;
    if (!dims_ok(dim_in, dim_hidden, dim_out, layers) || (x_plane_rows != 0 && x_plane_rows < n) ||
        (dx_plane_rows != 0 && dx_plane_rows < n) ||
        (planes_half && (x_plane_rows == 0 || dx_plane_rows == 0 || !half_mode)) || W1 == nullptr || b1 == nullptr ||
        W3 == nullptr || b3 == nullptr || dW1 == nullptr || db1 == nullptr || dW3 == nullptr || db3 == nullptr ||
        (layers == 3 && (W2 == nullptr || b2 == nullptr || dW2 == nullptr || db2 == nullptr)))
        return (int)hipErrorInvalidValue;
    if (dxv == xv && dx_plane_rows != x_plane_rows) return (int)hipErrorInvalidValue;
    if (n == 0) return 0;
    const float *x = reinterpret_cast<const float *>(xv);
    float *dx = reinterpret_cast<float *>(dxv);
    const Weights w{W1, b1, W2, b2, W3, b3};
    const Grads g{dW1, db1, dW2, db2, dW3, db3};
    const int nth = (int)dim_hidden / 32;
    const dim3 grid(grid_for(n, MI3D_TUNE(MI3D_T_MLP_WGS_PER_CU, 2))), block(kWave * kWavesPerWG);
    hipStream_t st = as_stream(stream);
    const bool classic = nth == 2 && layers == 3 && dim_in == (uint32_t)DIN;
    if (half_mode && planes_half)
        MI3D_MLP_DISPATCH(launch_bwd, F16, true, nth, layers, grid, st, x, x_plane_rows, dout, n, dim_in, w, dx, dx_plane_rows, g);
    else if (half_mode)
        MI3D_MLP_DISPATCH(launch_bwd, F16, false, nth, layers, grid, st, x, x_plane_rows, dout, n, dim_in, w, dx, dx_plane_rows, g);
    else if (classic)
        hipLaunchKernelGGL((k_mlp_backward<F32, 1, 1, false>), grid, block, lds_bytes<F32>(B_ALL_COUNT), st, x, x_plane_rows, 0,
                           dout, n, w, dx, dx_plane_rows, g);
    else
        MI3D_MLP_DISPATCH(launch_bwd, F32, false, nth, layers, grid, st, x, x_plane_rows, dout, n, dim_in, w, dx, dx_plane_rows, g);
    return (int)hipGetLastError();
}

int mi3d_field_head_forward(const float *h, const float *x, const float *x2, uint32_t n, const float *offsets_host,
                            uint32_t P, float bound, float blob_density, float blob_radius, float epsilon, float *sigma,
                            float *albedo, float *normal, float *normal2, void *stream) {
    return mi3d_field_head_forward_counted(h, x, x2, n, nullptr, offsets_host, P, bound, blob_density, blob_radius, epsilon,
                                           sigma, albedo, normal, normal2, stream);
}

int mi3d_field_head_forward_counted(const float *h, const float *x, const float *x2, uint32_t n, const int32_t *count,
                                    const float *offsets_host, uint32_t P, float bound, float blob_density,
                                    float blob_radius, float epsilon, float *sigma, float *albedo, float *normal,
                                    float *normal2, void *stream) {
    if ((P != 7 && P != 13) || (P == 13 && (x2 == nullptr || normal2 == nullptr))) return (int)hipErrorInvalidValue;
    if (n == 0) return 0;
    const HeadArgs a = make_head_args(x, x2, offsets_host, P, bound, blob_density, blob_radius, epsilon);
    hipLaunchKernelGGL(k_head_forward, dim3((n + 255) / 256), dim3(256), 0, as_stream(stream),
                       reinterpret_cast<const float4 *>(h), a, n, sigma, albedo, normal, normal2, count);
    return (int)hipGetLastError();
}

int mi3d_field_head_backward(const float *h, const float *x, const float *x2, uint32_t n, const float *offsets_host,
                             uint32_t P, uint32_t P_active, float bound, float blob_density, float blob_radius,
                             float epsilon, const float *dsigma, const float *dalbedo, const float *dnormal,
                             const float *dnormal2, float *dh, void *stream) {
    if ((P != 7 && P != 13) || (P == 13 && x2 == nullptr)) return (int)hipErrorInvalidValue;
    if ((P_active != 1 && P_active != 7 && P_active != 13) || P_active > P) return (int)hipErrorInvalidValue;
    if (n == 0) return 0;
    const HeadArgs a = make_head_args(x, x2, offsets_host, P, bound, blob_density, blob_radius, epsilon);
    hipLaunchKernelGGL(k_head_backward, dim3((n + 255) / 256), dim3(256), 0, as_stream(stream),
                       reinterpret_cast<const float4 *>(h), a, n, P_active, dsigma, dalbedo, dnormal, dnormal2,
                       reinterpret_cast<float4 *>(dh));
    return (int)hipGetLastError();
}

}
```

### make-it-3d_amd/mi3d/_lib.py

```python
import ctypes as C
import os

import torch

_CSRC = os.path.join(os.path.dirname(os.path.dirname(os.path.abspath(__file__))), "csrc")
LIB_PATH = os.environ.get("MI3D_LIB", os.path.join(_CSRC, "libmi3d.so"))

_lib = None

vp, u32, i32, f32 = C.c_void_p, C.c_uint32, C.c_int32, C.c_float

_SIGNATURES = {
    "mi3d_near_far_from_aabb": [vp, vp, vp, u32, f32, vp, vp, vp],
    "mi3d_sph_from_ray": [vp, vp, f32, u32, vp, vp],
    "mi3d_morton3D": [vp, u32, vp, vp],
    "mi3d_morton3D_invert": [vp, u32, vp, vp],
    "mi3d_packbits": [vp, u32, f32, vp, vp],
    "mi3d_march_rays_train": [vp, vp, vp, f32, f32, u32, u32, u32, u32, u32, vp, vp, vp, vp, vp, vp, vp, vp, vp],
    "mi3d_march_zero_tail": [vp, u32, u32, vp, vp, vp, vp],
    "mi3d_composite_rays_train_forward": [vp, vp, vp, vp, u32, u32, f32, vp, vp, vp, vp],
    "mi3d_composite_rays_train_backward": [vp, vp, vp, vp, vp, vp, vp, vp, u32, u32, f32, vp, vp, vp],
    "mi3d_composite_rays_train_backward_depth": [vp, vp, vp, vp, vp, vp, vp, vp, vp, vp, u32, u32, f32, vp, vp, vp],
    "mi3d_composite_sdf_rays_train_forward": [vp, vp, vp, vp, u32, u32, f32, vp, vp, vp, vp],
    "mi3d_composite_sdf_rays_train_backward": [vp, vp, vp, vp, vp, vp, vp, vp, u32, u32, f32, vp, vp, vp],
    "mi3d_march_rays": [u32, u32, vp, vp, vp, vp, f32, f32, u32, u32, u32, vp, vp, vp, vp, vp, vp, vp, vp],
    "mi3d_composite_rays": [u32, u32, f32, vp, vp, vp, vp, vp, vp, vp, vp, vp, vp, vp],
    "mi3d_composite_sdf_rays": [u32, u32, f32, vp, vp, vp, vp, vp, vp, vp, vp, vp],
    "mi3d_infer_begin": [vp, vp, u32, u32, vp],
    "mi3d_march_rays_ctl": [vp, u32, vp, vp, vp, vp, f32, f32, u32, u32, u32, vp, vp, vp, vp, vp, vp, vp],
    "mi3d_composite_rays_ctl": [vp, u32, f32, vp, vp, vp, vp, vp, vp, vp, vp, vp, vp, vp],
    "mi3d_compact_alive_ctl": [vp, vp, vp, u32, u32, u32, vp],
    "mi3d_infer_begin2": [vp, vp, u32, u32, u32, u32, vp],
    "mi3d_march_rays_compact_ctl": [vp, u32, vp, vp, vp, vp, f32, f32, u32, u32, u32, vp, vp, u32, vp, vp, vp, vp, vp, vp, vp],
    "mi3d_composite_rays_compact_ctl": [vp, u32, f32, vp, vp, vp, vp, vp, vp, vp, vp, vp, vp, vp, vp, vp],
    "mi3d_compact_alive_ctl2": [vp, vp, vp, u32, u32, vp],
    "mi3d_hashgrid_forward": [vp, u32, vp, u32, u32, f32, u32, vp, vp],
    "mi3d_hashgrid_backward": [vp, u32, vp, u32, u32, f32, u32, vp, vp],
    "mi3d_grid_encode_points": [vp, vp, u32, vp, vp, u32, u32, f32, vp, u32, u32, f32, u32, vp, vp],
    "mi3d_grid_scatter_points": [vp, vp, u32, vp, vp, u32, u32, f32, vp, u32, u32, f32, u32, f32, vp, vp],
    "mi3d_grid_encode_points_planes": [vp, vp, u32, vp, u32, u32, f32, vp, u32, u32, f32, u32, f32, vp, i32, vp],
    "mi3d_grid_scatter_binned": [vp, vp, u32, vp, u32, u32, f32, vp, i32, u32, u32, f32, u32, f32, vp, C.c_size_t, vp, vp],
    "mi3d_grid_scatter_binned_plus": [vp, vp, u32, vp, u32, u32, f32, vp, vp, i32, u32, u32, f32, u32, f32, vp, C.c_size_t,
                                      vp, vp],
    "mi3d_grid_encode_points_planes_counted": [vp, vp, u32, vp, vp, u32, u32, f32, vp, u32, u32, f32, u32, f32, vp, i32, vp],
    "mi3d_grid_encode_plan": [u32, f32, f32, u32, u32, f32, u32, vp, vp],
    "mi3d_grid_scatter_plan": [u32, u32, f32, f32, u32, u32, f32, u32, C.c_size_t, vp],
    "mi3d_grid_level_routes": [u32, u32, f32, u32, i32, vp],
    "mi3d_mlp_supported": [u32, u32, u32, u32],
    "mi3d_mlp_forward": [vp, u32, i32, u32, vp, vp, vp, vp, vp, vp, u32, u32, u32, i32, vp, vp],
    "mi3d_mlp_forward_counted": [vp, u32, i32, u32, vp, u32, vp, vp, vp, vp, vp, vp, u32, u32, u32, i32, vp, vp],
    "mi3d_mlp_backward": [vp, u32, i32, vp, u32, vp, vp, vp, vp, vp, vp, u32, u32, u32, i32, vp, u32, vp, vp, vp, vp, vp, vp, vp],
    "mi3d_field_head_forward": [vp, vp, vp, u32, vp, u32, f32, f32, f32, f32, vp, vp, vp, vp, vp],
    "mi3d_field_head_forward_counted": [vp, vp, vp, u32, vp, vp, u32, f32, f32, f32, f32, vp, vp, vp, vp, vp],
    "mi3d_field_head_backward": [vp, vp, vp, u32, vp, u32, u32, f32, f32, f32, f32, vp, vp, vp, vp, vp, vp],
    "mi3d_sumsq_accumulate": [vp, C.c_size_t, vp, vp],
    "mi3d_adan_step": [vp, vp, vp, vp, vp, vp, C.c_size_t, vp, f32, f32, i32, f32, f32, f32, f32, f32, f32, f32, f32, f32,
                       i32, vp],
    "mi3d_points_rasterize": [vp, u32, u32, u32, f32, u32, vp, C.c_size_t, vp, vp, vp, vp],
    "mi3d_points_composite_forward": [vp, vp, u32, u32, u32, vp, u32, C.c_double, vp, vp],
    "mi3d_points_composite_backward": [vp, vp, u32, u32, u32, vp, u32, C.c_double, vp, vp],
    "mi3d_mc_count": [vp, u32, u32, u32, f32, vp, C.c_size_t, vp, vp],
    "mi3d_mc_scan": [u32, u32, u32, vp, C.c_size_t, vp, vp],
    "mi3d_mc_emit": [vp, u32, u32, u32, f32, vp, vp, vp, C.c_size_t, vp, vp, C.c_uint64, vp, C.c_uint64, vp],
    "mi3d_atlas_uv": [C.c_uint64, u32, vp, vp],
    "mi3d_atlas_positions": [vp, C.c_uint64, vp, C.c_uint64, u32, u32, u32, u32, vp, vp, vp, vp],
    "mi3d_texture_pack": [vp, vp, u32, u32, u32, vp, vp],
    "mi3d_groupnorm_stats": [vp, u32, u32, u32, u32, vp, vp],
    "mi3d_groupnorm_act_forward": [vp, vp, vp, vp, u32, u32, u32, u32, f32, i32, vp, vp, vp, vp],
    "mi3d_groupnorm_act_backward_sums": [vp, vp, vp, vp, vp, vp, u32, u32, u32, u32, i32, vp, vp],
    "mi3d_groupnorm_act_backward": [vp, vp, vp, vp, vp, vp, vp, u32, u32, u32, u32, i32, vp, vp],
    "mi3d_pc_unproject": [vp, vp, u32, u32, vp, vp, vp, C.c_size_t, vp, C.c_uint64, vp, vp],
    "mi3d_pc_project": [vp, C.c_uint64, vp, vp, vp, vp, vp],
    "mi3d_pc_zmin": [vp, C.c_uint64, vp, vp, u32, u32, vp, vp],
    "mi3d_pc_visible": [vp, C.c_uint64, vp, vp, u32, u32, vp, vp, vp],
    "mi3d_box_morph": [vp, vp, u32, u32, u32, u32, i32, vp],
    "mi3d_pc_cano_filter": [vp, C.c_uint64, vp, vp, vp, u32, u32, vp, vp],
    "mi3d_pc_colour": [vp, C.c_uint64, vp, vp, vp, u32, u32, vp, vp],
    "mi3d_canny_classify": [vp, u32, u32, i32, i32, vp, vp, vp],
    "mi3d_canny_hysteresis": [vp, u32, u32, u32, vp, vp],
}

_LATE_SIGNATURES = {
    "mi3d_mc_workspace": ([u32, u32, u32], C.c_size_t),
    "mi3d_mc_case": ([u32, C.POINTER(C.c_int8)], C.c_int),
    "mi3d_atlas_cell": ([C.c_uint64, u32], u32),
    "mi3d_groupnorm_chunks": ([u32], u32),
    "mi3d_pc_unproject_workspace": ([u32, u32], C.c_size_t),
}


class Mi3dError(RuntimeError):
    pass


def lib():
    global _lib
    if _lib is None:
        if not os.path.exists(LIB_PATH):
            raise Mi3dError(f"{LIB_PATH} not found - build it first: python -c 'import __graft_entry__ as g; g.build()'")
        _lib = C.CDLL(LIB_PATH)
        for name, args in _SIGNATURES.items():
            fn = getattr(_lib, name)
            fn.argtypes = args
            fn.restype = C.c_int
        _lib.mi3d_abi_version.restype = C.c_int
        _lib.mi3d_last_error_string.restype = C.c_char_p
        _lib.mi3d_last_error_string.argtypes = [C.c_int]
        _lib.mi3d_hashgrid_levels.restype = u32
        _lib.mi3d_hashgrid_levels.argtypes = [u32, u32, f32, u32, vp, vp, vp]
        _lib.mi3d_grid_scatter_binned_workspace.restype = C.c_size_t
        _lib.mi3d_grid_scatter_binned_workspace.argtypes = [u32, u32, f32, f32, u32, u32, f32, u32]
        _lib.mi3d_points_rasterize_workspace.restype = C.c_size_t
        _lib.mi3d_points_rasterize_workspace.argtypes = [u32, u32, u32, f32]
        for name, (args, res) in _LATE_SIGNATURES.items():
            fn = getattr(_lib, name)
            fn.argtypes, fn.restype = args, res
    return _lib


def declare(name, argtypes, restype=C.c_int):
    fn = getattr(lib(), name)
    fn.argtypes, fn.restype = argtypes, restype
    return fn


def call(name, *args):
    err = getattr(lib(), name)(*args)
    if err != 0:
        raise Mi3dError(f"{name} failed: hipError {err} ({lib().mi3d_last_error_string(err).decode()})")


def launch(name, t, *args):
    with torch.cuda.device(t.device):
        call(name, *args, stream(t))


def stream(t=None):
    dev = t.device if isinstance(t, torch.Tensor) and t.is_cuda else None
    return C.c_void_p(torch.cuda.current_stream(dev).cuda_stream)


def on(t):
    return torch.cuda.device(t.device)


def ptr(t):
    return C.c_void_p(t.data_ptr()) if t is not None else C.c_void_p(0)


def dev_f32(t, name, shape_last=None):
    if not isinstance(t, torch.Tensor):
        raise TypeError(f"{name} must be a torch.Tensor")
    if not t.is_cuda:
        raise Mi3dError(f"{name} must live on the GPU (got {t.device})")
    if t.dtype != torch.float32:
        raise Mi3dError(f"{name} must be float32 (got {t.dtype})")
    if not t.is_contiguous():
        raise Mi3dError(f"{name} must be contiguous")
    if shape_last is not None and (t.dim() == 0 or t.shape[-1] != shape_last):
        raise Mi3dError(f"{name} must have last dimension {shape_last} (got {tuple(t.shape)})")
    return t


def dev_typed(t, name, dtype):
    if not t.is_cuda or t.dtype != dtype or not t.is_contiguous():
        raise Mi3dError(f"{name} must be a contiguous {dtype} GPU tensor (got {t.dtype} on {t.device})")
    return t
```

### make-it-3d_amd/mi3d/field_ops.py

```python
import ctypes as C
import os
import threading

import numpy as np
import torch
from torch.autograd import Function

from . import _lib as L
from . import grid_ops
from . import mlp_ops

WORKSPACE_CAP_BYTES = int(float(os.environ.get("MI3D_SCATTER_WORKSPACE_GB", "33")) * (1 << 30))


PLACED_MIN_BYTES = 8 << 30
PLACEMENT_TRIALS = int(os.environ.get("MI3D_SCATTER_PLACEMENT_TRIALS", "0"))
_ARENA_LOCK = threading.RLock()
_ARENAS = {}
_ARENA_LAST_USE = {}
PLACEMENT_LOG = []


def release_scatter_arena(device=None):
    with _ARENA_LOCK:
        for k in [k for k in _ARENAS if device is None or k == torch.device(device).index]:
            del _ARENAS[k]
            _ARENA_LAST_USE.pop(k, None)


def _alloc(want):
    failed = False
    while want > 0 and not (failed and want < (64 << 20)):
        try:
            return torch.empty(want, dtype=torch.uint8, device="cuda")
        except torch.cuda.OutOfMemoryError:
            failed = True
            want //= 2
    return None


def scatter_workspace(device, needed, cap=None, trial=None):
    cap = WORKSPACE_CAP_BYTES if cap is None else int(cap)
    gib = 1 << 30
    device = torch.device(device)
    held = _ARENAS.get(device.index)
    free, _ = torch.cuda.mem_get_info(device)
    cached = torch.cuda.memory_reserved(device) - torch.cuda.memory_allocated(device)
    room = free + cached + (held.numel() if held is not None else 0)
    want = min((int(needed) + gib - 1) // gib * gib if needed > gib else int(needed), cap, int(0.8 * room))
    with torch.cuda.device(device), _ARENA_LOCK:
        if want < PLACED_MIN_BYTES:
            return _alloc(want)
        if held is not None and held.numel() >= want:
            return held[:want]
        if held is not None:
            del _ARENAS[device.index], held
        n_try = 1
        trials = PLACEMENT_TRIALS if PLACEMENT_TRIALS > 0 else (7 if want < (40 << 30) else 4)
        if trial is not None and trials > 1:
            torch.cuda.empty_cache()
            free, _ = torch.cuda.mem_get_info(device)
            n_try = max(1, min(trials, int(0.9 * free) // want))
        gap = 0
        if n_try > 1:
            gap = max(0, (int(0.9 * free) - n_try * want) // n_try) >> 28 << 28
        cands, times, spacers = [], [], []
        for _ in range(n_try):
            if gap:
                spacers.append(_alloc(gap))
            c = _alloc(want)
            if c is None or (cands and c.numel() < cands[0].numel()):
                break
            cands.append(c)
        del spacers
        if not cands:
            return None
        if len(cands) > 1:
            for c in cands:
                trial(c)
                torch.cuda.synchronize(device)
                e0, e1 = torch.cuda.Event(enable_timing=True), torch.cuda.Event(enable_timing=True)
                e0.record()
                trial(c)
                e1.record()
                torch.cuda.synchronize(device)
                times.append(e0.elapsed_time(e1))
            best = min(range(len(cands)), key=lambda i: times[i])
            PLACEMENT_LOG.append({"device": device.index, "bytes": cands[0].numel(), "candidates_ms": [round(t, 2) for t in times],
                                  "kept": best})
            keep = cands[best]
            del cands, c
            _ARENAS[device.index] = keep
            torch.cuda.empty_cache()
        else:
            _ARENAS[device.index] = cands[0]
        held = _ARENAS[device.index]
        return held[:want] if held.numel() >= want else held


def scatter_binned(x, x2, offsets, P0, bound, dplanes, cfg, step, n_params, workspace_bytes=None, extra0=None):
    offs, offs_p = grid_ops._offs_arg(offsets)
    P, n = offs.shape[0], x.shape[0]
    if dplanes.dtype not in (torch.float32, torch.float16) or not dplanes.is_cuda or not dplanes.is_contiguous():
        raise L.Mi3dError("dplanes must be a contiguous float32 / float16 GPU tensor")
    if dplanes.numel() != cfg["n_levels"] * n * P * 2:
        raise L.Mi3dError(f"dplanes has {dplanes.numel()} elements, expected [L={cfg['n_levels']}][{P * n}][2]")
    if extra0 is not None and (extra0.dtype != dplanes.dtype or not extra0.is_cuda or not extra0.is_contiguous()
                               or extra0.numel() != cfg["n_levels"] * n * 2 or extra0.device != dplanes.device):
        raise L.Mi3dError(f"extra0 must be contiguous {dplanes.dtype} planes [L={cfg['n_levels']}][{n}][2] on the same GPU")
    grad = torch.zeros(n_params, dtype=torch.float32, device=x.device)
    lib = L.lib()

    def launch(ws, planes, out):
        L.call("mi3d_grid_scatter_binned_plus", L.ptr(x), L.ptr(x2), n, offs_p, int(P0), P, float(bound), L.ptr(planes),
               L.ptr(extra0), int(dplanes.dtype == torch.float16), cfg["n_levels"], cfg["base_resolution"],
               cfg["per_level_scale"], cfg["log2_hashmap_size"], float(step),
               L.ptr(ws), C.c_size_t(ws.numel() if ws is not None else 0), L.ptr(out), L.stream(x))

    st = {}

    def trial(cand):
        if "planes" not in st:
            st["planes"] = torch.empty_like(dplanes).uniform_(-1.0, 1.0)
            st["out"] = torch.zeros_like(grad)
        with L.on(x):
            launch(cand, st["planes"], st["out"])

    ws = None
    if workspace_bytes != 0 and n > 0:
        needed = lib.mi3d_grid_scatter_binned_workspace(n, P, float(bound), float(step), cfg["n_levels"],
                                                        cfg["base_resolution"], cfg["per_level_scale"],
                                                        cfg["log2_hashmap_size"])
        if needed:
            try:
                ws = scatter_workspace(x.device, needed, workspace_bytes, trial=trial)
            except TypeError:
                ws = scatter_workspace(x.device, needed, workspace_bytes)
        st.clear()
    with L.on(x):
        placed = ws is not None and ws.numel() >= PLACED_MIN_BYTES
        if placed:
            cur = torch.cuda.current_stream(x.device)
            last = _ARENA_LAST_USE.get(x.device.index)
            if last is not None:
                cur.wait_event(last)
        grid_ops._timed("scatter", lambda: launch(ws, dplanes, grad), n * P)
        if placed:
            _ARENA_LAST_USE[x.device.index] = cur.record_event()
    return grad


def _forward_encode_mlp(params, ws, x, x2, offs, offs_p, P0, bound, cfg, half_mode, step=0.0, count=None):
    P, n = offs.shape[0], x.shape[0]
    pdt = torch.float16 if half_mode else torch.float32
    feats = torch.empty(cfg["n_levels"], P * n, 2, dtype=pdt, device=x.device)
    grid_ops._timed("encode", lambda: L.call(
        "mi3d_grid_encode_points_planes_counted", L.ptr(x), L.ptr(x2), n, L.ptr(count), offs_p, int(P0), P, float(bound),
        L.ptr(params), cfg["n_levels"], cfg["base_resolution"], cfg["per_level_scale"], cfg["log2_hashmap_size"],
        float(step), L.ptr(feats), int(bool(half_mode)), L.stream(x)), n * P)
    dims = (ws[0].shape[1], ws[0].shape[0], ws[4].shape[0])
    h = torch.empty(P * n, dims[2], dtype=torch.float32, device=x.device)
    grid_ops._timed("mlp_fwd", lambda: L.call(
        "mi3d_mlp_forward_counted", L.ptr(feats), P * n, int(bool(half_mode)), P * n, L.ptr(count), max(n, 1),
        *[L.ptr(t) for t in ws], *dims, int(half_mode), L.ptr(h), L.stream(x)), n * P)
    return feats, h, dims


def _last_pass_through_graph():
    try:
        return not bool(torch._C._autograd._get_current_graph_task_keep_graph())
    except Exception:
        return False


def _backward_mlp(dh, feats, ws, dims, x, cfg, half_mode, P_active, in_place=False):
    n = x.shape[0]
    rows, plane_rows = P_active * n, feats.shape[1]
    if in_place and rows == plane_rows and feats.is_contiguous():
        dplanes = feats
    else:
        dplanes = torch.empty(cfg["n_levels"], rows, 2, dtype=feats.dtype, device=x.device)
    grads = [None if t is None else torch.zeros_like(t) for t in ws]
    grid_ops._timed("mlp_bwd", lambda: L.call(
        "mi3d_mlp_backward", L.ptr(feats), plane_rows, int(feats.dtype == torch.float16), L.ptr(dh), rows,
        *[L.ptr(t) for t in ws], *dims, int(half_mode),
        L.ptr(dplanes), rows, *[L.ptr(g) for g in grads], L.stream(x)), rows)
    return dplanes, grads


def _scatter_planes(dplanes, x, x2, offs, P0, bound, cfg, step, n_params, P_active, extra0=None):
    n = x.shape[0]
    rows = P_active * n
    if grid_ops.CENSUS is not None:
        nz = (dplanes != 0).any(-1).view(dplanes.shape[0], P_active, n)
        if extra0 is not None:
            nz[:, 0] |= (extra0 != 0).any(-1)
        per_sample = nz.any(1)
        tiles = per_sample[:, :n - n % 64].view(per_sample.shape[0], -1, 64).any(-1)
        grid_ops.CENSUS.append({
            "P_active": int(P_active), "rows": int(rows), "with_deferred_point0": extra0 is not None,
            "nonzero_pairs_per_level": nz.sum((1, 2)),
            "samples_with_any_nonzero_point_per_level": per_sample.float().mean(1),
            "tiles64_with_any_nonzero_per_level": tiles.float().mean(1),
            "samples_nonzero_on_any_level": per_sample.any(0).float().mean(),
            "nonzero_fraction_per_point": nz.float().mean((0, 2))})
        del nz, per_sample, tiles
    if grid_ops.DENSIFY:
        tiny = 2.0 ** -24 if dplanes.dtype == torch.float16 else 1e-30
        grid_ops._timed("densify", lambda: dplanes.masked_fill_(dplanes == 0, tiny), rows)
    return scatter_binned(x, x2 if P_active > P0 else None, offs[:P_active], min(P0, P_active), bound, dplanes, cfg, step,
                          n_params, extra0=extra0)


def _backward_mlp_scatter(dh, feats, ws, dims, x, x2, offs, P0, bound, cfg, step, n_params, half_mode, P_active):
    dplanes, grads = _backward_mlp(dh, feats, ws, dims, x, cfg, half_mode, P_active)
    return _scatter_planes(dplanes, x, x2, offs, P0, bound, cfg, step, n_params, P_active), grads



def _accumulates_into_grad(param):
    try:
        node = param.__dict__.get("_mi3d_acc_node")
        if node is None:
            with torch.enable_grad():
                node = param.expand_as(param).grad_fn.next_functions[0][0]
            param.__dict__["_mi3d_acc_node"] = node
        return bool(torch._C._will_engine_execute_node(node))
    except AttributeError as e:
        _warn_once(f"torch._C._will_engine_execute_node unavailable ({e}): the point-0 deferral is off, every backward "
                   f"pass scatters on its own (about +10 ms per C2 step)")
        return False
    except Exception:
        return False


_WARNED = set()


def _warn_once(msg):
    if msg not in _WARNED:
        _WARNED.add(msg)
        import warnings
        warnings.warn(msg, RuntimeWarning, stacklevel=3)


def _may_defer(param, P, P_active):
    if not (grid_ops.deferral_allowed() and isinstance(param, grid_ops.GridParameter) and P_active == 1 and P > 1):
        return False
    if getattr(param, "_post_accumulate_grad_hooks", None):
        return False
    try:
        keep = torch._C._autograd._get_current_graph_task_keep_graph()
    except AttributeError as e:
        _warn_once(f"torch._C._autograd._get_current_graph_task_keep_graph unavailable ({e}): the point-0 deferral is "
                   f"off, every backward pass scatters on its own (about +10 ms per C2 step)")
        return False
    except Exception:
        return False
    return bool(keep) and _accumulates_into_grad(param)


def _park(param, key, item):
    pend = param.__dict__.setdefault("_mi3d_pending", [])
    older = [it for it in pend if it["key"] == key]
    if older:
        flush_pending(param, key)
    if len(pend) >= 2:
        flush_pending(param)
    item["key"] = key
    item["stream"] = torch.cuda.current_stream(item["x"].device)
    item["event"] = item["stream"].record_event()
    pend.append(item)


def _find_parked(param, key):
    pend = None if param is None else param.__dict__.get("_mi3d_pending")
    for it in pend or ():
        if it["key"] == key:
            cur = torch.cuda.current_stream(it["x"].device)
            cur.wait_event(it["event"])
            if it.get("stream") is not None and it["stream"] != cur:
                it["dplanes"].record_stream(cur)
            return it
    return None


def _consume_parked(param, item):
    pend = None if param is None else param.__dict__.get("_mi3d_pending")
    if pend and item is not None:
        pend[:] = [it for it in pend if it is not item]


@torch.no_grad()
def flush_pending(param, key=None):
    pend = param.__dict__.get("_mi3d_pending")
    if not pend:
        return
    items = [it for it in pend if key is None or it["key"] == key]
    for it in items:
        x = it["x"]
        with L.on(x):
            cur = torch.cuda.current_stream(x.device)
            cur.wait_event(it["event"])
            if it.get("stream") is not None and it["stream"] != cur:
                it["dplanes"].record_stream(cur)
            g = _scatter_planes(it["dplanes"], x, None, it["offs"], it["P0"], it["bound"], it["cfg"], it["step"],
                                it["n_params"], 1)
        pend[:] = [other for other in pend if other is not it]
        real = torch.Tensor.grad.__get__(param)
        if real is None:
            torch.Tensor.grad.__set__(param, g.view_as(param))
        else:
            real.add_(g.view_as(real))


class _FieldStencil(Function):

    @staticmethod
    @torch.amp.custom_fwd(device_type="cuda", cast_inputs=torch.float32)
    def forward(ctx, params, W1, b1, W2, b2, W3, b3, x, x2, offsets, P0, bound, cfg, step, half_mode):
        x = L.dev_f32(x.contiguous().view(-1, 3), "x", 3)
        if x2 is not None:
            x2 = L.dev_f32(x2.contiguous().view(-1, 3), "x2", 3)
        params = L.dev_f32(params, "params")
        ws = mlp_ops._weights((W1, b1, W2, b2, W3, b3))
        offs, offs_p = grid_ops._offs_arg(offsets)
        with L.on(x):
            feats, h, dims = _forward_encode_mlp(params, ws, x, x2, offs, offs_p, P0, bound, cfg, half_mode, step)
        ctx.save_for_backward(x, x2 if x2 is not None else x, feats, *ws)
        ctx.meta = (offs, int(P0), float(bound), cfg, float(step), x2 is not None, params.numel(), dims,
                    int(half_mode))
        return h

    @staticmethod
    @torch.amp.custom_bwd(device_type="cuda")
    def backward(ctx, dh):
        x, x2, feats, *ws = ctx.saved_tensors
        offs, P0, bound, cfg, step, has_x2, n_params, dims, half_mode = ctx.meta
        dh = L.dev_f32(dh.float().contiguous(), "dh", dims[2])
        with L.on(x):
            gp, grads = _backward_mlp_scatter(dh, feats, ws, dims, x, x2 if has_x2 else None, offs, P0, bound, cfg,
                                              step, n_params, half_mode, offs.shape[0])
        return (gp, *grads, None, None, None, None, None, None, None, None)


def _half_mode(half_mode):
    if half_mode is None:
        return torch.is_autocast_enabled("cuda") and torch.get_autocast_dtype("cuda") == torch.float16
    return bool(half_mode)


def field_stencil(params, layers, x, offsets, cfg, bound=1.0, x2=None, P0=None, step=0.0, half_mode=None):
    P = np.asarray(offsets).reshape(-1, 3).shape[0]
    if P0 is None:
        P0 = P
    return _FieldStencil.apply(params, *mlp_ops.layer_args(layers), x, x2, offsets, P0, bound, cfg, step,
                               _half_mode(half_mode))


def _head_forward(h, x, x2, offs, offs_p, bound, blob_density, blob_radius, epsilon, count=None, half_mode=False):
    P, n, dev = offs.shape[0], x.shape[0], x.device
    alloc = torch.empty if count is None else torch.zeros
    sigma = alloc(n, dtype=torch.float32, device=dev)
    albedo = alloc(n, 3, dtype=torch.float32, device=dev)
    normal = alloc(n, 3, dtype=torch.float32, device=dev)
    normal2 = alloc(n, 3, dtype=torch.float32, device=dev) if P == 13 else None
    grid_ops._timed("head_fwd", lambda: L.call(
        "mi3d_field_head_forward_counted", L.ptr(h), L.ptr(x), L.ptr(x2), n, L.ptr(count), offs_p, P, float(bound),
        float(blob_density), float(blob_radius), float(epsilon), L.ptr(sigma), L.ptr(albedo), L.ptr(normal),
        L.ptr(normal2), L.stream(x)), n)
    if half_mode:
        albedo.copy_(albedo.to(torch.float16))
    return sigma, albedo, normal, normal2


def _head_backward(h, x, x2, offs, bound, blob_density, blob_radius, epsilon, grads, P_active):
    _, offs_p = grid_ops._offs_arg(offs)
    n, P = x.shape[0], offs.shape[0]
    g = [None if t is None else L.dev_f32(t.float().contiguous(), "grad") for t in grads]
    g += [None] * (4 - len(g))
    dh = torch.empty(P_active * n, 4, dtype=torch.float32, device=x.device)
    grid_ops._timed("head_bwd", lambda: L.call(
        "mi3d_field_head_backward", L.ptr(h), L.ptr(x), L.ptr(x2), n, offs_p, P, int(P_active), float(bound),
        float(blob_density), float(blob_radius), float(epsilon), L.ptr(g[0]), L.ptr(g[1]), L.ptr(g[2]), L.ptr(g[3]),
        L.ptr(dh), L.stream(x)), n)
    return dh


def _active_points(P, grads):
    if P == 13 and len(grads) > 3 and grads[3] is not None:
        return 13
    if len(grads) > 2 and grads[2] is not None:
        return 7
    return 1


class _FieldHead(Function):

    @staticmethod
    @torch.amp.custom_fwd(device_type="cuda", cast_inputs=torch.float32)
    def forward(ctx, h, x, x2, offsets, bound, blob_density, blob_radius, epsilon):
        offs, offs_p = grid_ops._offs_arg(offsets)
        P = offs.shape[0]
        x = L.dev_f32(x.contiguous().view(-1, 3), "x", 3)
        n = x.shape[0]
        h = L.dev_f32(h.contiguous().view(P * n, 4), "h", 4)
        if x2 is not None:
            x2 = L.dev_f32(x2.contiguous().view(-1, 3), "x2", 3)
        with L.on(x):
            sigma, albedo, normal, normal2 = _head_forward(h, x, x2, offs, offs_p, bound, blob_density, blob_radius,
                                                           epsilon)
        ctx.save_for_backward(h, x, x2 if x2 is not None else x)
        ctx.meta = (offs, float(bound), float(blob_density), float(blob_radius), float(epsilon), x2 is not None)
        ctx.set_materialize_grads(False)
        if normal2 is None:
            return sigma, albedo, normal
        return sigma, albedo, normal, normal2

    @staticmethod
    @torch.amp.custom_bwd(device_type="cuda")
    def backward(ctx, *grads):
        h, x, x2 = ctx.saved_tensors
        offs, bound, blob_density, blob_radius, epsilon, has_x2 = ctx.meta
        P, n = offs.shape[0], x.shape[0]
        P_active = _active_points(P, grads)
        with L.on(x):
            dh = _head_backward(h, x, x2 if has_x2 else None, offs, bound, blob_density, blob_radius, epsilon, grads,
                                P_active)
        if P_active < P:
            dh = torch.cat([dh, dh.new_zeros((P - P_active) * n, 4)], 0)
        return dh, None, None, None, None, None, None, None


def field_head(h, x, offsets, bound, blob_density, blob_radius, x2=None, epsilon=grid_ops.EPS):
    out = _FieldHead.apply(h, x, x2, offsets, bound, blob_density, blob_radius, epsilon)
    return out if len(out) == 4 else (*out, None)


class _Field(Function):

    @staticmethod
    @torch.amp.custom_fwd(device_type="cuda", cast_inputs=torch.float32)
    def forward(ctx, params, W1, b1, W2, b2, W3, b3, x, x2, offsets, P0, bound, cfg, step, half_mode, blob_density,
                blob_radius, epsilon):
        x = L.dev_f32(x.contiguous().view(-1, 3), "x", 3)
        if x2 is not None:
            x2 = L.dev_f32(x2.contiguous().view(-1, 3), "x2", 3)
        params = L.dev_f32(params, "params")
        ws = mlp_ops._weights((W1, b1, W2, b2, W3, b3))
        offs, offs_p = grid_ops._offs_arg(offsets)
        if offs.shape[0] not in (7, 13):
            raise L.Mi3dError("the fused field takes the 7- or 13-point stencil")
        with L.on(x):
            feats, h, dims = _forward_encode_mlp(params, ws, x, x2, offs, offs_p, P0, bound, cfg, half_mode, step)
            sigma, albedo, normal, normal2 = _head_forward(h, x, x2, offs, offs_p, bound, blob_density, blob_radius,
                                                           epsilon, half_mode=half_mode)
        ctx.save_for_backward(x, x2 if x2 is not None else x, feats, h, *ws)
        ctx.meta = (offs, int(P0), float(bound), cfg, float(step), x2 is not None, params.numel(), dims,
                    int(half_mode), float(blob_density), float(blob_radius), float(epsilon))
        ctx.param_ref = params if isinstance(params, grid_ops.GridParameter) else None
        ctx.forward_key = object()
        ctx.set_materialize_grads(False)
        if normal2 is None:
            return sigma, albedo, normal
        return sigma, albedo, normal, normal2

    @staticmethod
    @torch.amp.custom_bwd(device_type="cuda")
    def backward(ctx, *grads):
        x, x2, feats, h, *ws = ctx.saved_tensors
        (offs, P0, bound, cfg, step, has_x2, n_params, dims, half_mode, blob_density, blob_radius,
         epsilon) = ctx.meta
        none = (None,) * 18
        if all(g is None for g in grads):
            return none
        P_active = _active_points(offs.shape[0], grads)
        param = getattr(ctx, "param_ref", None)
        with L.on(x):
            dh = _head_backward(h, x, x2 if has_x2 else None, offs, bound, blob_density, blob_radius, epsilon, grads,
                                P_active)
            dplanes, wg = _backward_mlp(dh, feats, ws, dims, x, cfg, half_mode, P_active,
                                        in_place=grid_ops.INPLACE_GRAD_PLANES and P_active == offs.shape[0]
                                        and _last_pass_through_graph())
            del dh
            if _may_defer(param, offs.shape[0], P_active):
                _park(param, ctx.forward_key, dict(dplanes=dplanes, x=x, offs=offs, P0=P0, bound=bound, cfg=cfg,
                                                   step=step, n_params=n_params))
                gp = None
            else:
                parked = _find_parked(param, ctx.forward_key) if P_active > 1 else None
                gp = _scatter_planes(dplanes, x, x2 if has_x2 else None, offs, P0, bound, cfg, step, n_params, P_active,
                                     extra0=None if parked is None else parked["dplanes"])
                _consume_parked(param, parked)
        return (gp, *wg, *none[:11])


@torch.no_grad()
def field_rows(params, layers, x, offsets, cfg, bound, blob_density, blob_radius, count, step=0.0, half_mode=None,
               epsilon=grid_ops.EPS):
    x = L.dev_f32(x.contiguous().view(-1, 3).float(), "x", 3)
    params = L.dev_f32(params.detach(), "params")
    ws = mlp_ops._weights([None if t is None else t.detach() for t in mlp_ops.layer_args(layers)])
    offs, offs_p = grid_ops._offs_arg(offsets)
    if offs.shape[0] != 7:
        raise L.Mi3dError("field_rows takes the 7-point stencil")
    count = L.dev_typed(count, "count", torch.int32)
    with L.on(x):
        hm = _half_mode(half_mode)
        _, h, _ = _forward_encode_mlp(params, ws, x, None, offs, offs_p, 7, bound, cfg, hm, step, count)
        sigma, albedo, normal, _ = _head_forward(h, x, None, offs, offs_p, bound, blob_density, blob_radius, epsilon, count,
                                                 half_mode=hm)
    return sigma, albedo, normal


def field(params, layers, x, offsets, cfg, bound, blob_density, blob_radius, x2=None, P0=None, step=0.0,
          half_mode=None, epsilon=grid_ops.EPS):
    P = np.asarray(offsets).reshape(-1, 3).shape[0]
    if P0 is None:
        P0 = P
    out = _Field.apply(params, *mlp_ops.layer_args(layers), x, x2, offsets, P0, bound, cfg, step,
                       _half_mode(half_mode), blob_density, blob_radius, epsilon)
    return out if len(out) == 4 else (*out, None)
```

### make-it-3d_amd/mi3d/network.py

```python
import numpy as np
import torch
import torch.nn as nn
import torch.nn.functional as F

import tinycudann as tcnn

from . import field_ops, grid_ops, mlp_ops
from .renderer import NeRFRenderer, safe_normalize


class _TruncExp(torch.autograd.Function):

    @staticmethod
    @torch.amp.custom_fwd(device_type="cuda", cast_inputs=torch.float32)
    def forward(ctx, x):
        ctx.save_for_backward(x)
        return torch.exp(x)

    @staticmethod
    @torch.amp.custom_bwd(device_type="cuda")
    def backward(ctx, g):
        (x,) = ctx.saved_tensors
        return g * torch.exp(x.clamp(max=15))


trunc_exp = _TruncExp.apply


class MLP(nn.Module):

    def __init__(self, dim_in, dim_out, dim_hidden, num_layers, bias=True):
        super().__init__()
        self.dim_in, self.dim_out, self.dim_hidden, self.num_layers = dim_in, dim_out, dim_hidden, num_layers
        self.net = nn.ModuleList([
            nn.Linear(dim_in if l == 0 else dim_hidden, dim_out if l == num_layers - 1 else dim_hidden, bias=bias)
            for l in range(num_layers)])

    def fused_ok(self, x):
        return (x.is_cuda and all(l.bias is not None for l in self.net)
                and mlp_ops.supported(self.dim_in, self.dim_hidden, self.dim_out, self.num_layers))

    def forward(self, x):
        if self.fused_ok(x):
            return mlp_ops.fused_mlp(x, self.net)
        if x.is_cuda:
            raise mlp_ops.L.Mi3dError(
                f"MLP {self.dim_in} -> {self.num_layers - 1} x {self.dim_hidden} -> {self.dim_out} (bias "
                f"{all(l.bias is not None for l in self.net)}) is not covered by the matrix-core kernels "
                f"(dim_in even and <= 32, hidden 32 or 64, 2 or 3 layers, 4 outputs, biased)")
        for l, layer in enumerate(self.net):
            x = layer(x)
            if l != self.num_layers - 1:
                x = F.relu(x, inplace=True)
        return x


class NeRFNetwork(NeRFRenderer):
    def __init__(self, opt, bg_color=None, num_layers=3, hidden_dim=64, num_layers_bg=2, hidden_dim_bg=64,
                 n_levels=16, log2_hashmap_size=19, base_resolution=16, per_level_scale=None):
        super().__init__(opt)
        self.num_layers, self.hidden_dim = num_layers, hidden_dim
        if per_level_scale is None:
            per_level_scale = np.exp2(np.log2(2048 * self.bound / 16) / (16 - 1))
        self.encoder = tcnn.Encoding(n_input_dims=3, encoding_config={
            "otype": "HashGrid", "n_levels": n_levels, "n_features_per_level": 2,
            "log2_hashmap_size": log2_hashmap_size, "base_resolution": base_resolution,
            "per_level_scale": per_level_scale}, dtype=torch.float32)
        self.sigma_net = MLP(self.encoder.n_output_dims, 4, hidden_dim, num_layers, bias=True)
        if self.bg_radius > 0:
            raise NotImplementedError("bg_radius > 0 (background network) is not on Make-It-3D's path (main.py:54)")
        self.bg_net = None
        if bg_color is not None:
            bg64 = F.interpolate(bg_color, size=64, mode="bicubic", align_corners=True)
            self.register_buffer("bg_color", bg64.permute(0, 2, 3, 1).reshape(-1, 3).clone(), persistent=False)
        else:
            self.register_buffer("bg_color", torch.rand((4096, 3)), persistent=False)

    def gaussian(self, x):
        d = (x ** 2).sum(-1)
        return self.opt.blob_density * torch.exp(-d / (2 * self.opt.blob_radius ** 2))

    @staticmethod
    def _sigmoid(h):
        if h.is_cuda and field_ops._half_mode(None):
            h = h.to(torch.float16)
        return torch.sigmoid(h)

    def _head(self, h, x):
        sigma = trunc_exp(h[..., 0] + self.gaussian(x))
        albedo = self._sigmoid(h[..., 1:])
        return sigma, albedo

    def _encode(self, x, offsets, x2=None, P0=None, step=0.0):
        return grid_ops.encode_points(self.encoder.params, x, offsets, self.encoder.cfg, float(self.bound), x2, P0,
                                      step)

    _CENTER = np.zeros((1, 3), np.float32)

    def common_forward(self, x):
        x = x.reshape(-1, 3).float()
        return self._head(self.sigma_net(self._encode(x, self._CENTER)), x)

    def _stencil_sigma(self, x, offsets, x2=None, P0=None, step=0.0):
        n, P = x.shape[0], offsets.shape[0]
        if self.sigma_net.fused_ok(x) and self.encoder.cfg["n_levels"] * 2 == self.sigma_net.dim_in:
            h = field_ops.field_stencil(self.encoder.params, self.sigma_net.net, x, offsets, self.encoder.cfg,
                                        float(self.bound), x2, P0, step)
        else:
            h = self.sigma_net(self._encode(x, offsets, x2, P0, step))
        h = h.view(P, n, 4).transpose(0, 1)
        offs = torch.from_numpy(offsets).to(x.device)
        base = x.unsqueeze(1).expand(n, P, 3)
        if x2 is not None:
            base = torch.cat([base[:, :P0], x2.unsqueeze(1).expand(n, P - P0, 3)], 1)
        pts = (base + offs).clamp(-self.bound, self.bound)
        sigma = trunc_exp(h[..., 0] + self.gaussian(pts))
        return sigma, h

    @staticmethod
    def _normal_from(s6, epsilon=grid_ops.EPS):
        g = torch.stack([0.5 * (s6[:, 0] - s6[:, 1]) / epsilon, 0.5 * (s6[:, 2] - s6[:, 3]) / epsilon,
                         0.5 * (s6[:, 4] - s6[:, 5]) / epsilon], -1)
        return torch.nan_to_num(safe_normalize(-g))

    def finite_difference_normal(self, x, epsilon=grid_ops.EPS):
        offs, _ = grid_ops.stencil_offsets(center=False)
        if epsilon != grid_ops.EPS:
            offs = offs / np.float32(grid_ops.EPS) * np.float32(epsilon)
        s6, _ = self._stencil_sigma(x.reshape(-1, 3).float(), offs)
        return -torch.stack([0.5 * (s6[:, 0] - s6[:, 1]) / epsilon, 0.5 * (s6[:, 2] - s6[:, 3]) / epsilon,
                             0.5 * (s6[:, 4] - s6[:, 5]) / epsilon], -1)

    def normal(self, x):
        return torch.nan_to_num(safe_normalize(self.finite_difference_normal(x)))

    def field_stencil(self, x, x2=None, step=0.0):
        x = x.reshape(-1, 3).float()
        offs, P0 = grid_ops.stencil_offsets(center=True, second=x2 is not None)
        if x.is_cuda and self.sigma_net.fused_ok(x) and self.encoder.cfg["n_levels"] * 2 == self.sigma_net.dim_in:
            return field_ops.field(self.encoder.params, self.sigma_net.net, x, offs, self.encoder.cfg, float(self.bound),
                                   self.opt.blob_density, self.opt.blob_radius, x2, P0 if x2 is not None else None, step)
        sig, h = self._stencil_sigma(x, offs, x2, P0 if x2 is not None else None, step)
        albedo = self._sigmoid(h[:, 0, 1:])
        normals = self._normal_from(sig[:, 1:7])
        normals_jitter = self._normal_from(sig[:, 7:13]) if x2 is not None else None
        return sig[:, 0], albedo, normals, normals_jitter

    def shade(self, albedo, normal, light_d, ratio, shading, batch_rows=None):
        if shading == "albedo" or (normal.shape[0] if batch_rows is None else batch_rows) >= 1e6:
            return albedo
        lambertian = ratio + (1 - ratio) * (normal @ light_d).clamp(min=0.1)
        if shading == "textureless":
            return lambertian.unsqueeze(-1).repeat(1, 3)
        if shading == "normal":
            return (normal + 1) / 2
        return albedo * lambertian.unsqueeze(-1)

    def forward(self, x, d, l=None, ratio=1, shading="albedo"):
        rows = getattr(self, "_infer_rows", None)
        if (rows is not None and not torch.is_grad_enabled() and x.is_cuda and self.sigma_net.fused_ok(x)
                and self.encoder.cfg["n_levels"] * 2 == self.sigma_net.dim_in):
            offs, _ = grid_ops.stencil_offsets(center=True, second=False)
            sigma, albedo, normal = field_ops.field_rows(self.encoder.params, self.sigma_net.net, x.reshape(-1, 3), offs,
                                                         self.encoder.cfg, float(self.bound), self.opt.blob_density,
                                                         self.opt.blob_radius, rows)
            return sigma, self.shade(albedo, normal, l, ratio, shading, getattr(self, "_infer_shade_rows", None)), normal
        sigma, albedo, normal, _ = self.field_stencil(x)
        return sigma, self.shade(albedo, normal, l, ratio, shading), normal

    def density(self, x):
        sigma, albedo = self.common_forward(x)
        return {"sigma": sigma, "albedo": albedo}

    def background(self, d):
        raise NotImplementedError("no background network (bg_radius <= 0 on this path)")

    def get_params(self, lr):
        return [{"params": self.encoder.parameters(), "lr": lr * 10}, {"params": self.sigma_net.parameters(), "lr": lr}]
```

Measured before the change: 10.96.

## Store only the density channel for stencil neighbour rows in training field path

Adds a compact training path for the fused field. The MLP forward writes full 4-channel outputs only for centre rows and a single sigma channel for the 12 stencil neighbour rows, and the head and MLP backward kernels read and write that compact tail. The aim is to cut the f32x4 output and gradient traffic for neighbour points, which only need density, to about a quarter. The cost is extra branching on the row slot in the kernels and a new autograd function that runs only in training when x2 is present.

```diff
diff --git a/include/mi3d.h b/include/mi3d.h
--- a/include/mi3d.h
+++ b/include/mi3d.h
@@ -170,6 +170,28 @@
                              const float *dnormal2, float *dh, void *stream);
 
 
+int mi3d_mlp_forward_compact(const void *x, uint32_t x_plane_rows, int planes_half, uint32_t n, uint32_t n_stride,
+                             const float *W1, const float *b1, const float *W2, const float *b2, const float *W3,
+                             const float *b3, uint32_t dim_in, uint32_t dim_hidden, uint32_t dim_out, int half_mode,
+                             float *h0, float *hs, void *stream);
+int mi3d_mlp_backward_compact(const void *x, uint32_t x_plane_rows, int planes_half, const float *dh0, const float *dhs,
+                              uint32_t n, uint32_t n_stride, const float *W1, const float *b1, const float *W2,
+                              const float *b2, const float *W3, const float *b3, uint32_t dim_in, uint32_t dim_hidden,
+                              uint32_t dim_out, int half_mode, void *dx, uint32_t dx_plane_rows, float *dW1, float *db1,
+                              float *dW2, float *db2, float *dW3, float *db3, void *stream);
+int mi3d_field_head_forward_train(const float *h0, const float *hs, const float *x, const float *x2, uint32_t n,
+                                  const float *offsets_host, uint32_t P, float bound, float blob_density,
+                                  float blob_radius, float epsilon, int round_albedo, float *sigma, float *albedo,
+                                  float *normal, float *normal2, void *stream);
+int mi3d_field_head_backward_train(const float *h0, const float *hs, const float *x, const float *x2, uint32_t n,
+                                   const float *offsets_host, uint32_t P, uint32_t P_active, float bound,
+                                   float blob_density, float blob_radius, float epsilon, const float *dsigma,
+                                   const float *dalbedo, const float *dnormal, const float *dnormal2, float *dh0,
+                                   float *dhs, void *stream);
+int mi3d_field_tail_layout(uint32_t n, uint32_t P, uint64_t *h0_floats, uint64_t *hs_floats, uint32_t *buffer,
+                           uint64_t *offset);
+
+
 int mi3d_sumsq_accumulate(const float *x, size_t n, float *acc, void *stream);
 int mi3d_adan_step(float *param, float *grad, float *exp_avg, float *exp_avg_sq, float *exp_avg_diff,
                    float *neg_pre_grad, size_t count, const float *grad_sumsq, float max_grad_norm, float clip_eps,
diff --git a/make-it-3d_amd/csrc/field.hip b/make-it-3d_amd/csrc/field.hip
--- a/make-it-3d_amd/csrc/field.hip
+++ b/make-it-3d_amd/csrc/field.hip
@@ -283,6 +283,23 @@
 __device__ __forceinline__ f32x4 load_dout_raw(const float *__restrict__ dout, size_t row, size_t n) {
     return *reinterpret_cast<const f32x4 *>(dout + (row < n ? row : n - 1) * DOUT);
 }
+struct TailSlot {
+    uint32_t neighbour;
+    size_t index;
+};
+__host__ __device__ inline TailSlot tail_slot(size_t row, size_t n) {
+    return row < n ? TailSlot{0u, row} : TailSlot{1u, row - n};
+}
+template <class T> __host__ __device__ __forceinline__ const T &only(const T &t) { return t; }
+struct DoutTail {
+    const float *dhs;
+    uint32_t n0;
+};
+__device__ __forceinline__ f32x4 load_dout_raw(const float *__restrict__ dh0, size_t row, size_t n, const DoutTail &tail) {
+    const TailSlot t = tail_slot(row < n ? row : n - 1, tail.n0);
+    if (t.neighbour) return f32x4{tail.dhs[t.index], 0.f, 0.f, 0.f};
+    return *reinterpret_cast<const f32x4 *>(dh0 + t.index * DOUT);
+}
 template <class P> __device__ __forceinline__ typename P::KB dout_kb(const f32x4 &t, bool keep) {
     typename P::KB k;
 #pragma unroll
@@ -306,11 +323,12 @@
     float *dW1, *db1, *dW2, *db2, *dW3, *db3;
 };
 
-template <class P, int U, int WPS, bool HP>
+template <class P, int U, int WPS, bool HP, class... TAIL>
 __global__ __launch_bounds__(kWave *kWavesPerWG, WPS) void k_mlp_backward(const float *x, uint32_t x_planes,
                                                                            int , const float *__restrict__ dout,
                                                                            uint32_t n, Weights w, float *dx,
-                                                                           uint32_t dx_planes, Grads g) {
+                                                                           uint32_t dx_planes, Grads g, TAIL... tail) {
+    static_assert(sizeof...(TAIL) <= 1, "at most the compact rows' tail");
     extern __shared__ __attribute__((aligned(16))) char lds[];
     float *bias = reinterpret_cast<float *>(lds + (size_t)B_ALL_COUNT * block_bytes<P>());
     build_blocks<P>(lds, bias, w, B_ALL_COUNT);
@@ -342,7 +360,7 @@
         const size_t r0 = ((size_t)wave + (size_t)u * n_waves) * 32 + p;
         if constexpr (HP) load_rows_half(x, r0, n, h, x_planes, rawh[u]);
         else load_rows_raw(x, r0, n, h, x_planes, raw[u]);
-        dor[u] = load_dout_raw(dout, r0, n);
+        dor[u] = load_dout_raw(dout, r0, n, tail...);
     }
     for (uint32_t tile = wave; tile < n_tiles; tile += U * n_waves) {
         size_t row[U];
@@ -362,7 +380,7 @@
                 const size_t rn = ((size_t)tile + (size_t)(U + u) * n_waves) * 32 + p;
                 if constexpr (HP) load_rows_half(x, rn, n, h, x_planes, rawh[u]);
                 else load_rows_raw(x, rn, n, h, x_planes, raw[u]);
-                dor[u] = load_dout_raw(dout, rn, n);
+                dor[u] = load_dout_raw(dout, rn, n, tail...);
             }
         }
 
@@ -779,11 +797,13 @@
     }
 }
 
-template <class P, int NTH, int LAYERS, bool HP>
+template <class P, int NTH, int LAYERS, bool HP, class... HS>
 __global__ __launch_bounds__(kWave *kWavesPerWG, 2) void k_mlp_fwd_g(const float *__restrict__ x, uint32_t x_planes,
                                                                         uint32_t n, uint32_t din, Weights w,
                                                                         float *__restrict__ out,
-                                                                        const int32_t *__restrict__ count, uint32_t n_stride) {
+                                                                        const int32_t *__restrict__ count, uint32_t n_stride,
+                                                                        HS... hs) {
+    static_assert(sizeof...(HS) <= 1, "at most the compact rows' second buffer");
     using B = Blk<NTH, LAYERS>;
     using KB = typename P::KB;
     extern __shared__ __attribute__((aligned(16))) char lds[];
@@ -846,17 +866,28 @@
 #pragma unroll
         for (int tk = 0; tk < NTH; ++tk) P::mma(acc, blk(B::W3 + tk), HL[tk]);
         if (row < n && h == 0 && live) {
-            f32x4 o = {P::round(acc[0]), P::round(acc[1]), P::round(acc[2]), P::round(acc[3])};
-            __builtin_nontemporal_store(o, reinterpret_cast<f32x4 *>(out + row * DOUT));
-        }
-    }
-}
-
-template <class P, int NTH, int LAYERS, bool HP, bool FULL>
+            if constexpr (sizeof...(HS) != 0) {
+                const TailSlot t = tail_slot(row, n_stride);
+                if (t.neighbour) {
+                    __builtin_nontemporal_store(P::round(acc[0]), only(hs...) + t.index);
+                } else {
+                    f32x4 o = {P::round(acc[0]), P::round(acc[1]), P::round(acc[2]), P::round(acc[3])};
+                    __builtin_nontemporal_store(o, reinterpret_cast<f32x4 *>(out + t.index * DOUT));
+                }
+            } else {
+                f32x4 o = {P::round(acc[0]), P::round(acc[1]), P::round(acc[2]), P::round(acc[3])};
+                __builtin_nontemporal_store(o, reinterpret_cast<f32x4 *>(out + row * DOUT));
+            }
+        }
+    }
+}
+
+template <class P, int NTH, int LAYERS, bool HP, bool FULL, class... TAIL>
 __global__ __launch_bounds__(kWave *kWavesPerWG, 2) void k_mlp_bwd_g(const float *x, uint32_t x_planes,
                                                                         const float *__restrict__ dout, uint32_t n,
                                                                         uint32_t din, Weights w, float *dx,
-                                                                        uint32_t dx_planes, Grads g) {
+                                                                        uint32_t dx_planes, Grads g, TAIL... tail) {
+    static_assert(sizeof...(TAIL) <= 1, "at most the compact rows' tail");
     using B = Blk<NTH, LAYERS>;
     using KB = typename P::KB;
     constexpr int H = 32 * NTH;
@@ -913,7 +944,7 @@
         const size_t r0 = (size_t)wave * 32 + p;
         if constexpr (HP) load_rows_half_g<FULL && P::kLdsTranspose>(x, r0, n, h, x_planes, last_plane, rawh);
         else load_rows_raw_g(x, r0, n, h, x_planes, din, raw);
-        dor = load_dout_raw(dout, r0, n);
+        dor = load_dout_raw(dout, r0, n, tail...);
     }
     for (uint32_t tile = wave; tile < n_tiles; tile += n_waves) {
         const size_t row = (size_t)tile * 32 + p;
@@ -929,7 +960,7 @@
                 const size_t rn = ((size_t)tile + n_waves) * 32 + p;
                 if constexpr (HP) load_rows_half_g<FULL && P::kLdsTranspose>(x, rn, n, P::kLdsTranspose ? ht : h, xp, last_plane, rawh);
                 else load_rows_raw_g(x, rn, n, P::kLdsTranspose ? ht : h, xp, din, raw);
-                dor = load_dout_raw(dout, rn, n);
+                dor = load_dout_raw(dout, rn, n, tail...);
             }
         };
         constexpr bool late_prefetch = P::kLdsTranspose && HP;
@@ -1149,26 +1180,49 @@
     }
 }
 
+struct HeadTail {
+    const float *hs;
+    int round_albedo;
+};
+struct HeadGradTail {
+    const float *hs;
+    float *dhs;
+};
+__device__ __forceinline__ float head_x(const float4 *__restrict__ h, size_t row, size_t) { return h[row].x; }
+template <class T> __device__ __forceinline__ float head_x(const float4 *__restrict__, size_t row, size_t n, const T &t) {
+    return t.hs[tail_slot(row, n).index];
+}
+__device__ __forceinline__ float head_albedo(float v) { return v; }
+__device__ __forceinline__ float head_albedo(float v, const HeadTail &t) { return t.round_albedo ? (float)(_Float16)v : v; }
+__device__ __forceinline__ void head_put(float4 *__restrict__ dh, size_t row, size_t, float du) {
+    dh[row] = make_float4(du, 0.f, 0.f, 0.f);
+}
+__device__ __forceinline__ void head_put(float4 *__restrict__, size_t row, size_t n, float du, const HeadGradTail &t) {
+    t.dhs[tail_slot(row, n).index] = du;
+}
+
+template <class... TAIL>
 __global__ void k_head_forward(const float4 *__restrict__ h, HeadArgs a, uint32_t n, float *__restrict__ sigma,
                                float *__restrict__ albedo, float *__restrict__ normal, float *__restrict__ normal2,
-                               const int32_t *__restrict__ count) {
+                               const int32_t *__restrict__ count, TAIL... tail) {
+    static_assert(sizeof...(TAIL) <= 1, "at most the compact rows' tail");
     const uint32_t s = blockIdx.x * blockDim.x + threadIdx.x;
     if (s >= n || (count && (int32_t)s >= *count)) return;
     float bx[3] = {a.x[(size_t)s * 3], a.x[(size_t)s * 3 + 1], a.x[(size_t)s * 3 + 2]};
     const float4 h0 = h[s];
     sigma[s] = expf(h0.x + head_gauss(a, bx, 0));
-    albedo[(size_t)s * 3] = 1.0f / (1.0f + expf(-h0.y));
-    albedo[(size_t)s * 3 + 1] = 1.0f / (1.0f + expf(-h0.z));
-    albedo[(size_t)s * 3 + 2] = 1.0f / (1.0f + expf(-h0.w));
+    albedo[(size_t)s * 3] = head_albedo(1.0f / (1.0f + expf(-h0.y)), tail...);
+    albedo[(size_t)s * 3 + 1] = head_albedo(1.0f / (1.0f + expf(-h0.z)), tail...);
+    albedo[(size_t)s * 3 + 2] = head_albedo(1.0f / (1.0f + expf(-h0.w)), tail...);
     float sg[6], nn[3], v[3], c;
 #pragma unroll
-    for (uint32_t p = 0; p < 6; ++p) sg[p] = expf(h[(size_t)(1 + p) * n + s].x + head_gauss(a, bx, 1 + p));
+    for (uint32_t p = 0; p < 6; ++p) sg[p] = expf(head_x(h, (size_t)(1 + p) * n + s, n, tail...) + head_gauss(a, bx, 1 + p));
     head_normal(sg, a.inv_2eps, nn, v, c);
     normal[(size_t)s * 3] = nn[0]; normal[(size_t)s * 3 + 1] = nn[1]; normal[(size_t)s * 3 + 2] = nn[2];
     if (a.P == 13) {
         float b2[3] = {a.x2[(size_t)s * 3], a.x2[(size_t)s * 3 + 1], a.x2[(size_t)s * 3 + 2]};
 #pragma unroll
-        for (uint32_t p = 0; p < 6; ++p) sg[p] = expf(h[(size_t)(7 + p) * n + s].x + head_gauss(a, b2, 7 + p));
+        for (uint32_t p = 0; p < 6; ++p) sg[p] = expf(head_x(h, (size_t)(7 + p) * n + s, n, tail...) + head_gauss(a, b2, 7 + p));
         head_normal(sg, a.inv_2eps, nn, v, c);
         normal2[(size_t)s * 3] = nn[0]; normal2[(size_t)s * 3 + 1] = nn[1]; normal2[(size_t)s * 3 + 2] = nn[2];
     }
@@ -1199,10 +1253,12 @@
     }
 }
 
+template <class... TAIL>
 __global__ void k_head_backward(const float4 *__restrict__ h, HeadArgs a, uint32_t n, uint32_t P_active,
                                 const float *__restrict__ dsigma, const float *__restrict__ dalbedo,
                                 const float *__restrict__ dnormal, const float *__restrict__ dnormal2,
-                                float4 *__restrict__ dh) {
+                                float4 *__restrict__ dh, TAIL... tail) {
+    static_assert(sizeof...(TAIL) <= 1, "at most the compact rows' tail");
     const uint32_t s = blockIdx.x * blockDim.x + threadIdx.x;
     if (s >= n) return;
     float bx[3] = {a.x[(size_t)s * 3], a.x[(size_t)s * 3 + 1], a.x[(size_t)s * 3 + 2]};
@@ -1217,21 +1273,21 @@
     if (P_active < 7) return;
     float u[6], du[6], dn[3];
 #pragma unroll
-    for (uint32_t p = 0; p < 6; ++p) u[p] = h[(size_t)(1 + p) * n + s].x + head_gauss(a, bx, 1 + p);
+    for (uint32_t p = 0; p < 6; ++p) u[p] = head_x(h, (size_t)(1 + p) * n + s, n, tail...) + head_gauss(a, bx, 1 + p);
 #pragma unroll
     for (int d = 0; d < 3; ++d) dn[d] = dnormal ? dnormal[(size_t)s * 3 + d] : 0.f;
     head_normal_backward(u, a.inv_2eps, dn, du);
 #pragma unroll
-    for (uint32_t p = 0; p < 6; ++p) dh[(size_t)(1 + p) * n + s] = make_float4(du[p], 0.f, 0.f, 0.f);
+    for (uint32_t p = 0; p < 6; ++p) head_put(dh, (size_t)(1 + p) * n + s, n, du[p], tail...);
     if (a.P == 13 && P_active == 13) {
         float b2[3] = {a.x2[(size_t)s * 3], a.x2[(size_t)s * 3 + 1], a.x2[(size_t)s * 3 + 2]};
 #pragma unroll
-        for (uint32_t p = 0; p < 6; ++p) u[p] = h[(size_t)(7 + p) * n + s].x + head_gauss(a, b2, 7 + p);
+        for (uint32_t p = 0; p < 6; ++p) u[p] = head_x(h, (size_t)(7 + p) * n + s, n, tail...) + head_gauss(a, b2, 7 + p);
 #pragma unroll
         for (int d = 0; d < 3; ++d) dn[d] = dnormal2 ? dnormal2[(size_t)s * 3 + d] : 0.f;
         head_normal_backward(u, a.inv_2eps, dn, du);
 #pragma unroll
-        for (uint32_t p = 0; p < 6; ++p) dh[(size_t)(7 + p) * n + s] = make_float4(du[p], 0.f, 0.f, 0.f);
+        for (uint32_t p = 0; p < 6; ++p) head_put(dh, (size_t)(7 + p) * n + s, n, du[p], tail...);
     }
 }
 
@@ -1264,23 +1320,25 @@
            (layers == 2 || layers == 3);
 }
 
-template <class P, int NTH, int LAYERS, bool HP>
+template <class P, int NTH, int LAYERS, bool HP, class... HS>
 void launch_fwd(dim3 grid, hipStream_t st, const float *x, uint32_t x_planes, uint32_t n, uint32_t din, const Weights &w,
-                float *out, const int32_t *count, uint32_t n_stride) {
+                float *out, const int32_t *count, uint32_t n_stride, HS... hs) {
     using B = Blk<NTH, LAYERS>;
-    hipLaunchKernelGGL((k_mlp_fwd_g<P, NTH, LAYERS, HP>), grid, dim3(kWave * kWavesPerWG),
-                       lds_bytes_g<P>(B::FWD_COUNT, B::BIAS_TILES), st, x, x_planes, n, din, w, out, count, n_stride);
-}
-template <class P, int NTH, int LAYERS, bool HP>
+    hipLaunchKernelGGL((k_mlp_fwd_g<P, NTH, LAYERS, HP, HS...>), grid, dim3(kWave * kWavesPerWG),
+                       lds_bytes_g<P>(B::FWD_COUNT, B::BIAS_TILES), st, x, x_planes, n, din, w, out, count, n_stride, hs...);
+}
+template <class P, int NTH, int LAYERS, bool HP, class... TAIL>
 void launch_bwd(dim3 grid, hipStream_t st, const float *x, uint32_t x_planes, const float *dout, uint32_t n, uint32_t din,
-                const Weights &w, float *dx, uint32_t dx_planes, const Grads &g) {
+                const Weights &w, float *dx, uint32_t dx_planes, const Grads &g, TAIL... tail) {
     using B = Blk<NTH, LAYERS>;
     if (HP && P::kLdsTranspose && din == (uint32_t)DIN)
-        hipLaunchKernelGGL((k_mlp_bwd_g<P, NTH, LAYERS, HP, HP && P::kLdsTranspose>), grid, dim3(kWave * kWavesPerWG),
-                           lds_bytes_g<P>(B::ALL_COUNT, B::BIAS_TILES, true), st, x, x_planes, dout, n, din, w, dx, dx_planes, g);
+        hipLaunchKernelGGL((k_mlp_bwd_g<P, NTH, LAYERS, HP, HP && P::kLdsTranspose, TAIL...>), grid, dim3(kWave * kWavesPerWG),
+                           lds_bytes_g<P>(B::ALL_COUNT, B::BIAS_TILES, true), st, x, x_planes, dout, n, din, w, dx, dx_planes, g,
+                           tail...);
     else
-        hipLaunchKernelGGL((k_mlp_bwd_g<P, NTH, LAYERS, HP, false>), grid, dim3(kWave * kWavesPerWG),
-                           lds_bytes_g<P>(B::ALL_COUNT, B::BIAS_TILES, true), st, x, x_planes, dout, n, din, w, dx, dx_planes, g);
+        hipLaunchKernelGGL((k_mlp_bwd_g<P, NTH, LAYERS, HP, false, TAIL...>), grid, dim3(kWave * kWavesPerWG),
+                           lds_bytes_g<P>(B::ALL_COUNT, B::BIAS_TILES, true), st, x, x_planes, dout, n, din, w, dx, dx_planes, g,
+                           tail...);
 }
 #define MI3D_MLP_DISPATCH(FN, P, HP, nth, layers, ...)                     \
     do {                                                                   \
@@ -1290,25 +1348,11 @@
         else FN<P, 1, 2, HP>(__VA_ARGS__);                                 \
     } while (0)
 
-}
-
-extern "C" {
-
-int mi3d_mlp_supported(uint32_t dim_in, uint32_t dim_hidden, uint32_t dim_out, uint32_t num_layers) {
-    return dims_ok(dim_in, dim_hidden, dim_out, num_layers) ? 1 : 0;
-}
-
-int mi3d_mlp_forward(const void *xv, uint32_t x_plane_rows, int planes_half, uint32_t n, const float *W1, const float *b1, const float *W2, const float *b2,
-                     const float *W3, const float *b3, uint32_t dim_in, uint32_t dim_hidden, uint32_t dim_out,
-                     int half_mode, float *out, void *stream) {
-    return mi3d_mlp_forward_counted(xv, x_plane_rows, planes_half, n, nullptr, n ? n : 1u, W1, b1, W2, b2, W3, b3, dim_in,
-                                    dim_hidden, dim_out, half_mode, out, stream);
-}
-
-int mi3d_mlp_forward_counted(const void *xv, uint32_t x_plane_rows, int planes_half, uint32_t n, const int32_t *count,
-                             uint32_t n_stride, const float *W1, const float *b1, const float *W2, const float *b2,
-                             const float *W3, const float *b3, uint32_t dim_in, uint32_t dim_hidden, uint32_t dim_out,
-                             int half_mode, float *out, void *stream) {
+template <class... HS>
+int mlp_forward_any(const void *xv, uint32_t x_plane_rows, int planes_half, uint32_t n, const int32_t *count,
+                    uint32_t n_stride, const float *W1, const float *b1, const float *W2, const float *b2,
+                    const float *W3, const float *b3, uint32_t dim_in, uint32_t dim_hidden, uint32_t dim_out,
+                    int half_mode, float *out, void *stream, HS... hs) {
     if (n_stride == 0) return (int)hipErrorInvalidValue;
     const uint32_t layers = (W2 == nullptr && b2 == nullptr) ? 2u : 3u;
     if (!dims_ok(dim_in, dim_hidden, dim_out, layers) || (x_plane_rows != 0 && x_plane_rows < n) ||
@@ -1321,16 +1365,17 @@
     const int nth = (int)dim_hidden / 32;
     hipStream_t st = as_stream(stream);
     const dim3 grid(grid_for(n, MI3D_TUNE(MI3D_T_MLP_FWD_WGS_PER_CU, 5)));
-    if (half_mode && planes_half) MI3D_MLP_DISPATCH(launch_fwd, F16, true, nth, layers, grid, st, x, x_plane_rows, n, dim_in, w, out, count, n_stride);
-    else if (half_mode) MI3D_MLP_DISPATCH(launch_fwd, F16, false, nth, layers, grid, st, x, x_plane_rows, n, dim_in, w, out, count, n_stride);
-    else MI3D_MLP_DISPATCH(launch_fwd, F32, false, nth, layers, grid, st, x, x_plane_rows, n, dim_in, w, out, count, n_stride);
+    if (half_mode && planes_half) MI3D_MLP_DISPATCH(launch_fwd, F16, true, nth, layers, grid, st, x, x_plane_rows, n, dim_in, w, out, count, n_stride, hs...);
+    else if (half_mode) MI3D_MLP_DISPATCH(launch_fwd, F16, false, nth, layers, grid, st, x, x_plane_rows, n, dim_in, w, out, count, n_stride, hs...);
+    else MI3D_MLP_DISPATCH(launch_fwd, F32, false, nth, layers, grid, st, x, x_plane_rows, n, dim_in, w, out, count, n_stride, hs...);
     return (int)hipGetLastError();
 }
 
-int mi3d_mlp_backward(const void *xv, uint32_t x_plane_rows, int planes_half, const float *dout, uint32_t n, const float *W1, const float *b1,
-                      const float *W2, const float *b2, const float *W3, const float *b3, uint32_t dim_in,
-                      uint32_t dim_hidden, uint32_t dim_out, int half_mode, void *dxv, uint32_t dx_plane_rows, float *dW1, float *db1, float *dW2, float *db2, float *dW3, float *db3,
-                      void *stream) {
+template <class... TAIL>
+int mlp_backward_any(const void *xv, uint32_t x_plane_rows, int planes_half, const float *dout, uint32_t n, const float *W1,
+                     const float *b1, const float *W2, const float *b2, const float *W3, const float *b3, uint32_t dim_in,
+                     uint32_t dim_hidden, uint32_t dim_out, int half_mode, void *dxv, uint32_t dx_plane_rows, float *dW1,
+                     float *db1, float *dW2, float *db2, float *dW3, float *db3, void *stream, TAIL... tail) {
     const uint32_t layers = (W2 == nullptr && b2 == nullptr) ? 2u : 3u;
     if (!dims_ok(dim_in, dim_hidden, dim_out, layers) || (x_plane_rows != 0 && x_plane_rows < n) ||
         (dx_plane_rows != 0 && dx_plane_rows < n) ||
@@ -1349,15 +1394,65 @@
     hipStream_t st = as_stream(stream);
     const bool classic = nth == 2 && layers == 3 && dim_in == (uint32_t)DIN;
     if (half_mode && planes_half)
-        MI3D_MLP_DISPATCH(launch_bwd, F16, true, nth, layers, grid, st, x, x_plane_rows, dout, n, dim_in, w, dx, dx_plane_rows, g);
+        MI3D_MLP_DISPATCH(launch_bwd, F16, true, nth, layers, grid, st, x, x_plane_rows, dout, n, dim_in, w, dx, dx_plane_rows, g, tail...);
     else if (half_mode)
-        MI3D_MLP_DISPATCH(launch_bwd, F16, false, nth, layers, grid, st, x, x_plane_rows, dout, n, dim_in, w, dx, dx_plane_rows, g);
+        MI3D_MLP_DISPATCH(launch_bwd, F16, false, nth, layers, grid, st, x, x_plane_rows, dout, n, dim_in, w, dx, dx_plane_rows, g, tail...);
     else if (classic)
-        hipLaunchKernelGGL((k_mlp_backward<F32, 1, 1, false>), grid, block, lds_bytes<F32>(B_ALL_COUNT), st, x, x_plane_rows, 0,
-                           dout, n, w, dx, dx_plane_rows, g);
+        hipLaunchKernelGGL((k_mlp_backward<F32, 1, 1, false, TAIL...>), grid, block, lds_bytes<F32>(B_ALL_COUNT), st, x,
+                           x_plane_rows, 0, dout, n, w, dx, dx_plane_rows, g, tail...);
     else
-        MI3D_MLP_DISPATCH(launch_bwd, F32, false, nth, layers, grid, st, x, x_plane_rows, dout, n, dim_in, w, dx, dx_plane_rows, g);
+        MI3D_MLP_DISPATCH(launch_bwd, F32, false, nth, layers, grid, st, x, x_plane_rows, dout, n, dim_in, w, dx, dx_plane_rows, g, tail...);
     return (int)hipGetLastError();
+}
+
+}
+
+extern "C" {
+
+int mi3d_mlp_supported(uint32_t dim_in, uint32_t dim_hidden, uint32_t dim_out, uint32_t num_layers) {
+    return dims_ok(dim_in, dim_hidden, dim_out, num_layers) ? 1 : 0;
+}
+
+int mi3d_mlp_forward(const void *xv, uint32_t x_plane_rows, int planes_half, uint32_t n, const float *W1, const float *b1, const float *W2, const float *b2,
+                     const float *W3, const float *b3, uint32_t dim_in, uint32_t dim_hidden, uint32_t dim_out,
+                     int half_mode, float *out, void *stream) {
+    return mi3d_mlp_forward_counted(xv, x_plane_rows, planes_half, n, nullptr, n ? n : 1u, W1, b1, W2, b2, W3, b3, dim_in,
+                                    dim_hidden, dim_out, half_mode, out, stream);
+}
+
+int mi3d_mlp_forward_counted(const void *xv, uint32_t x_plane_rows, int planes_half, uint32_t n, const int32_t *count,
+                             uint32_t n_stride, const float *W1, const float *b1, const float *W2, const float *b2,
+                             const float *W3, const float *b3, uint32_t dim_in, uint32_t dim_hidden, uint32_t dim_out,
+                             int half_mode, float *out, void *stream) {
+    return mlp_forward_any(xv, x_plane_rows, planes_half, n, count, n_stride, W1, b1, W2, b2, W3, b3, dim_in, dim_hidden,
+                           dim_out, half_mode, out, stream);
+}
+
+int mi3d_mlp_forward_compact(const void *xv, uint32_t x_plane_rows, int planes_half, uint32_t n, uint32_t n_stride,
+                             const float *W1, const float *b1, const float *W2, const float *b2, const float *W3,
+                             const float *b3, uint32_t dim_in, uint32_t dim_hidden, uint32_t dim_out, int half_mode,
+                             float *h0, float *hs, void *stream) {
+    if (h0 == nullptr || (hs == nullptr && n > n_stride)) return (int)hipErrorInvalidValue;
+    return mlp_forward_any(xv, x_plane_rows, planes_half, n, nullptr, n_stride, W1, b1, W2, b2, W3, b3, dim_in, dim_hidden,
+                           dim_out, half_mode, h0, stream, hs);
+}
+
+int mi3d_mlp_backward(const void *xv, uint32_t x_plane_rows, int planes_half, const float *dout, uint32_t n, const float *W1, const float *b1,
+                      const float *W2, const float *b2, const float *W3, const float *b3, uint32_t dim_in,
+                      uint32_t dim_hidden, uint32_t dim_out, int half_mode, void *dxv, uint32_t dx_plane_rows, float *dW1, float *db1, float *dW2, float *db2, float *dW3, float *db3,
+                      void *stream) {
+    return mlp_backward_any(xv, x_plane_rows, planes_half, dout, n, W1, b1, W2, b2, W3, b3, dim_in, dim_hidden, dim_out,
+                            half_mode, dxv, dx_plane_rows, dW1, db1, dW2, db2, dW3, db3, stream);
+}
+
+int mi3d_mlp_backward_compact(const void *xv, uint32_t x_plane_rows, int planes_half, const float *dh0, const float *dhs,
+                              uint32_t n, uint32_t n_stride, const float *W1, const float *b1, const float *W2,
+                              const float *b2, const float *W3, const float *b3, uint32_t dim_in, uint32_t dim_hidden,
+                              uint32_t dim_out, int half_mode, void *dxv, uint32_t dx_plane_rows, float *dW1, float *db1,
+                              float *dW2, float *db2, float *dW3, float *db3, void *stream) {
+    if (n_stride == 0 || dh0 == nullptr || (dhs == nullptr && n > n_stride)) return (int)hipErrorInvalidValue;
+    return mlp_backward_any(xv, x_plane_rows, planes_half, dh0, n, W1, b1, W2, b2, W3, b3, dim_in, dim_hidden, dim_out,
+                            half_mode, dxv, dx_plane_rows, dW1, db1, dW2, db2, dW3, db3, stream, DoutTail{dhs, n_stride});
 }
 
 int mi3d_field_head_forward(const float *h, const float *x, const float *x2, uint32_t n, const float *offsets_host,
@@ -1374,8 +1469,22 @@
     if ((P != 7 && P != 13) || (P == 13 && (x2 == nullptr || normal2 == nullptr))) return (int)hipErrorInvalidValue;
     if (n == 0) return 0;
     const HeadArgs a = make_head_args(x, x2, offsets_host, P, bound, blob_density, blob_radius, epsilon);
-    hipLaunchKernelGGL(k_head_forward, dim3((n + 255) / 256), dim3(256), 0, as_stream(stream),
+    hipLaunchKernelGGL(k_head_forward<>, dim3((n + 255) / 256), dim3(256), 0, as_stream(stream),
                        reinterpret_cast<const float4 *>(h), a, n, sigma, albedo, normal, normal2, count);
+    return (int)hipGetLastError();
+}
+
+int mi3d_field_head_forward_train(const float *h0, const float *hs, const float *x, const float *x2, uint32_t n,
+                                  const float *offsets_host, uint32_t P, float bound, float blob_density,
+                                  float blob_radius, float epsilon, int round_albedo, float *sigma, float *albedo,
+                                  float *normal, float *normal2, void *stream) {
+    if ((P != 7 && P != 13) || (P == 13 && (x2 == nullptr || normal2 == nullptr))) return (int)hipErrorInvalidValue;
+    if (n == 0) return 0;
+    if (h0 == nullptr || hs == nullptr) return (int)hipErrorInvalidValue;
+    const HeadArgs a = make_head_args(x, x2, offsets_host, P, bound, blob_density, blob_radius, epsilon);
+    hipLaunchKernelGGL(k_head_forward<HeadTail>, dim3((n + 255) / 256), dim3(256), 0, as_stream(stream),
+                       reinterpret_cast<const float4 *>(h0), a, n, sigma, albedo, normal, normal2,
+                       static_cast<const int32_t *>(nullptr), HeadTail{hs, round_albedo});
     return (int)hipGetLastError();
 }
 
@@ -1387,10 +1496,40 @@
     if ((P_active != 1 && P_active != 7 && P_active != 13) || P_active > P) return (int)hipErrorInvalidValue;
     if (n == 0) return 0;
     const HeadArgs a = make_head_args(x, x2, offsets_host, P, bound, blob_density, blob_radius, epsilon);
-    hipLaunchKernelGGL(k_head_backward, dim3((n + 255) / 256), dim3(256), 0, as_stream(stream),
+    hipLaunchKernelGGL(k_head_backward<>, dim3((n + 255) / 256), dim3(256), 0, as_stream(stream),
                        reinterpret_cast<const float4 *>(h), a, n, P_active, dsigma, dalbedo, dnormal, dnormal2,
                        reinterpret_cast<float4 *>(dh));
     return (int)hipGetLastError();
 }
 
-}
+int mi3d_field_head_backward_train(const float *h0, const float *hs, const float *x, const float *x2, uint32_t n,
+                                   const float *offsets_host, uint32_t P, uint32_t P_active, float bound,
+                                   float blob_density, float blob_radius, float epsilon, const float *dsigma,
+                                   const float *dalbedo, const float *dnormal, const float *dnormal2, float *dh0,
+                                   float *dhs, void *stream) {
+    if ((P != 7 && P != 13) || (P == 13 && x2 == nullptr)) return (int)hipErrorInvalidValue;
+    if ((P_active != 1 && P_active != 7 && P_active != 13) || P_active > P) return (int)hipErrorInvalidValue;
+    if (n == 0) return 0;
+    if (h0 == nullptr || dh0 == nullptr || (P_active > 1 && (hs == nullptr || dhs == nullptr))) return (int)hipErrorInvalidValue;
+    const HeadArgs a = make_head_args(x, x2, offsets_host, P, bound, blob_density, blob_radius, epsilon);
+    hipLaunchKernelGGL(k_head_backward<HeadGradTail>, dim3((n + 255) / 256), dim3(256), 0, as_stream(stream),
+                       reinterpret_cast<const float4 *>(h0), a, n, P_active, dsigma, dalbedo, dnormal, dnormal2,
+                       reinterpret_cast<float4 *>(dh0), HeadGradTail{hs, dhs});
+    return (int)hipGetLastError();
+}
+
+int mi3d_field_tail_layout(uint32_t n, uint32_t P, uint64_t *h0_floats, uint64_t *hs_floats, uint32_t *buffer,
+                           uint64_t *offset) {
+    if (P == 0) return (int)hipErrorInvalidValue;
+    if (h0_floats) *h0_floats = (uint64_t)n * DOUT;
+    if (hs_floats) *hs_floats = (uint64_t)n * (P - 1);
+    if (buffer && offset)
+        for (size_t row = 0; row < (size_t)n * P; ++row) {
+            const TailSlot t = tail_slot(row, n);
+            buffer[row] = t.neighbour;
+            offset[row] = t.neighbour ? (uint64_t)t.index : (uint64_t)t.index * DOUT;
+        }
+    return 0;
+}
+
+}
diff --git a/make-it-3d_amd/mi3d/_lib.py b/make-it-3d_amd/mi3d/_lib.py
--- a/make-it-3d_amd/mi3d/_lib.py
+++ b/make-it-3d_amd/mi3d/_lib.py
@@ -53,6 +53,12 @@
     "mi3d_field_head_forward": [vp, vp, vp, u32, vp, u32, f32, f32, f32, f32, vp, vp, vp, vp, vp],
     "mi3d_field_head_forward_counted": [vp, vp, vp, u32, vp, vp, u32, f32, f32, f32, f32, vp, vp, vp, vp, vp],
     "mi3d_field_head_backward": [vp, vp, vp, u32, vp, u32, u32, f32, f32, f32, f32, vp, vp, vp, vp, vp, vp],
+    "mi3d_mlp_forward_compact": [vp, u32, i32, u32, u32, vp, vp, vp, vp, vp, vp, u32, u32, u32, i32, vp, vp, vp],
+    "mi3d_mlp_backward_compact": [vp, u32, i32, vp, vp, u32, u32, vp, vp, vp, vp, vp, vp, u32, u32, u32, i32, vp, u32, vp,
+                                  vp, vp, vp, vp, vp, vp],
+    "mi3d_field_head_forward_train": [vp, vp, vp, vp, u32, vp, u32, f32, f32, f32, f32, i32, vp, vp, vp, vp, vp],
+    "mi3d_field_head_backward_train": [vp, vp, vp, vp, u32, vp, u32, u32, f32, f32, f32, f32, vp, vp, vp, vp, vp, vp, vp],
+    "mi3d_field_tail_layout": [u32, u32, vp, vp, vp, vp],
     "mi3d_sumsq_accumulate": [vp, C.c_size_t, vp, vp],
     "mi3d_adan_step": [vp, vp, vp, vp, vp, vp, C.c_size_t, vp, f32, f32, i32, f32, f32, f32, f32, f32, f32, f32, f32, f32,
                        i32, vp],
diff --git a/make-it-3d_amd/mi3d/field_ops.py b/make-it-3d_amd/mi3d/field_ops.py
--- a/make-it-3d_amd/mi3d/field_ops.py
+++ b/make-it-3d_amd/mi3d/field_ops.py
@@ -150,7 +150,7 @@
     return grad
 
 
-def _forward_encode_mlp(params, ws, x, x2, offs, offs_p, P0, bound, cfg, half_mode, step=0.0, count=None):
+def _encode_planes(params, x, x2, offs, offs_p, P0, bound, cfg, half_mode, step=0.0, count=None):
     P, n = offs.shape[0], x.shape[0]
     pdt = torch.float16 if half_mode else torch.float32
     feats = torch.empty(cfg["n_levels"], P * n, 2, dtype=pdt, device=x.device)
@@ -158,6 +158,12 @@
         "mi3d_grid_encode_points_planes_counted", L.ptr(x), L.ptr(x2), n, L.ptr(count), offs_p, int(P0), P, float(bound),
         L.ptr(params), cfg["n_levels"], cfg["base_resolution"], cfg["per_level_scale"], cfg["log2_hashmap_size"],
         float(step), L.ptr(feats), int(bool(half_mode)), L.stream(x)), n * P)
+    return feats
+
+
+def _forward_encode_mlp(params, ws, x, x2, offs, offs_p, P0, bound, cfg, half_mode, step=0.0, count=None):
+    P, n = offs.shape[0], x.shape[0]
+    feats = _encode_planes(params, x, x2, offs, offs_p, P0, bound, cfg, half_mode, step, count)
     dims = (ws[0].shape[1], ws[0].shape[0], ws[4].shape[0])
     h = torch.empty(P * n, dims[2], dtype=torch.float32, device=x.device)
     grid_ops._timed("mlp_fwd", lambda: L.call(
@@ -437,6 +443,18 @@
     return out if len(out) == 4 else (*out, None)
 
 
+def _park_or_scatter(param, key, dplanes, x, x2, offs, P0, bound, cfg, step, n_params, P_active):
+    if _may_defer(param, offs.shape[0], P_active):
+        _park(param, key, dict(dplanes=dplanes, x=x, offs=offs, P0=P0, bound=bound, cfg=cfg, step=step,
+                               n_params=n_params))
+        return None
+    parked = _find_parked(param, key) if P_active > 1 else None
+    gp = _scatter_planes(dplanes, x, x2, offs, P0, bound, cfg, step, n_params, P_active,
+                         extra0=None if parked is None else parked["dplanes"])
+    _consume_parked(param, parked)
+    return gp
+
+
 class _Field(Function):
 
     @staticmethod
@@ -483,16 +501,126 @@
                                         in_place=grid_ops.INPLACE_GRAD_PLANES and P_active == offs.shape[0]
                                         and _last_pass_through_graph())
             del dh
-            if _may_defer(param, offs.shape[0], P_active):
-                _park(param, ctx.forward_key, dict(dplanes=dplanes, x=x, offs=offs, P0=P0, bound=bound, cfg=cfg,
-                                                   step=step, n_params=n_params))
-                gp = None
-            else:
-                parked = _find_parked(param, ctx.forward_key) if P_active > 1 else None
-                gp = _scatter_planes(dplanes, x, x2 if has_x2 else None, offs, P0, bound, cfg, step, n_params, P_active,
-                                     extra0=None if parked is None else parked["dplanes"])
-                _consume_parked(param, parked)
+            gp = _park_or_scatter(param, ctx.forward_key, dplanes, x, x2 if has_x2 else None, offs, P0, bound, cfg, step,
+                                  n_params, P_active)
         return (gp, *wg, *none[:11])
+
+
+
+def _forward_encode_mlp_compact(params, ws, x, x2, offs, offs_p, P0, bound, cfg, half_mode, step=0.0):
+    P, n = offs.shape[0], x.shape[0]
+    feats = _encode_planes(params, x, x2, offs, offs_p, P0, bound, cfg, half_mode, step)
+    dims = (ws[0].shape[1], ws[0].shape[0], ws[4].shape[0])
+    h0 = torch.empty(n, dims[2], dtype=torch.float32, device=x.device)
+    hs = torch.empty((P - 1) * n, dtype=torch.float32, device=x.device)
+    grid_ops._timed("mlp_fwd", lambda: L.call(
+        "mi3d_mlp_forward_compact", L.ptr(feats), P * n, int(bool(half_mode)), P * n, max(n, 1),
+        *[L.ptr(t) for t in ws], *dims, int(half_mode), L.ptr(h0), L.ptr(hs), L.stream(x)), n * P)
+    return feats, h0, hs, dims
+
+
+def _head_forward_train(h0, hs, x, x2, offs, offs_p, bound, blob_density, blob_radius, epsilon, half_mode=False):
+    P, n, dev = offs.shape[0], x.shape[0], x.device
+    sigma = torch.empty(n, dtype=torch.float32, device=dev)
+    albedo = torch.empty(n, 3, dtype=torch.float32, device=dev)
+    normal = torch.empty(n, 3, dtype=torch.float32, device=dev)
+    normal2 = torch.empty(n, 3, dtype=torch.float32, device=dev) if P == 13 else None
+    grid_ops._timed("head_fwd", lambda: L.call(
+        "mi3d_field_head_forward_train", L.ptr(h0), L.ptr(hs), L.ptr(x), L.ptr(x2), n, offs_p, P, float(bound),
+        float(blob_density), float(blob_radius), float(epsilon), int(bool(half_mode)), L.ptr(sigma), L.ptr(albedo),
+        L.ptr(normal), L.ptr(normal2), L.stream(x)), n)
+    return sigma, albedo, normal, normal2
+
+
+def _head_backward_train(h0, hs, x, x2, offs, bound, blob_density, blob_radius, epsilon, grads, P_active):
+    _, offs_p = grid_ops._offs_arg(offs)
+    n, P = x.shape[0], offs.shape[0]
+    g = [None if t is None else L.dev_f32(t.float().contiguous(), "grad") for t in grads]
+    g += [None] * (4 - len(g))
+    dh0 = torch.empty(n, 4, dtype=torch.float32, device=x.device)
+    dhs = torch.empty((P_active - 1) * n, dtype=torch.float32, device=x.device) if P_active > 1 else None
+    grid_ops._timed("head_bwd", lambda: L.call(
+        "mi3d_field_head_backward_train", L.ptr(h0), L.ptr(hs), L.ptr(x), L.ptr(x2), n, offs_p, P, int(P_active),
+        float(bound), float(blob_density), float(blob_radius), float(epsilon), L.ptr(g[0]), L.ptr(g[1]), L.ptr(g[2]),
+        L.ptr(g[3]), L.ptr(dh0), L.ptr(dhs), L.stream(x)), n)
+    return dh0, dhs
+
+
+def _backward_mlp_compact(dh0, dhs, feats, ws, dims, x, cfg, half_mode, P_active, in_place=False):
+    n = x.shape[0]
+    rows, plane_rows = P_active * n, feats.shape[1]
+    if in_place and rows == plane_rows and feats.is_contiguous():
+        dplanes = feats
+    else:
+        dplanes = torch.empty(cfg["n_levels"], rows, 2, dtype=feats.dtype, device=x.device)
+    grads = [None if t is None else torch.zeros_like(t) for t in ws]
+    grid_ops._timed("mlp_bwd", lambda: L.call(
+        "mi3d_mlp_backward_compact", L.ptr(feats), plane_rows, int(feats.dtype == torch.float16), L.ptr(dh0), L.ptr(dhs),
+        rows, max(n, 1), *[L.ptr(t) for t in ws], *dims, int(half_mode),
+        L.ptr(dplanes), rows, *[L.ptr(g) for g in grads], L.stream(x)), rows)
+    return dplanes, grads
+
+
+class _FieldTrain(Function):
+
+    @staticmethod
+    @torch.amp.custom_fwd(device_type="cuda", cast_inputs=torch.float32)
+    def forward(ctx, params, W1, b1, W2, b2, W3, b3, x, x2, offsets, P0, bound, cfg, step, half_mode, blob_density,
+                blob_radius, epsilon):
+        x = L.dev_f32(x.contiguous().view(-1, 3), "x", 3)
+        if x2 is not None:
+            x2 = L.dev_f32(x2.contiguous().view(-1, 3), "x2", 3)
+        params = L.dev_f32(params, "params")
+        ws = mlp_ops._weights((W1, b1, W2, b2, W3, b3))
+        offs, offs_p = grid_ops._offs_arg(offsets)
+        if offs.shape[0] not in (7, 13):
+            raise L.Mi3dError("the fused field takes the 7- or 13-point stencil")
+        with L.on(x):
+            feats, h0, hs, dims = _forward_encode_mlp_compact(params, ws, x, x2, offs, offs_p, P0, bound, cfg, half_mode,
+                                                              step)
+            sigma, albedo, normal, normal2 = _head_forward_train(h0, hs, x, x2, offs, offs_p, bound, blob_density,
+                                                                 blob_radius, epsilon, half_mode=half_mode)
+        ctx.save_for_backward(x, x2 if x2 is not None else x, feats, h0, hs, *ws)
+        ctx.meta = (offs, int(P0), float(bound), cfg, float(step), x2 is not None, params.numel(), dims,
+                    int(half_mode), float(blob_density), float(blob_radius), float(epsilon))
+        ctx.param_ref = params if isinstance(params, grid_ops.GridParameter) else None
+        ctx.forward_key = object()
+        ctx.set_materialize_grads(False)
+        if normal2 is None:
+            return sigma, albedo, normal
+        return sigma, albedo, normal, normal2
+
+    @staticmethod
+    @torch.amp.custom_bwd(device_type="cuda")
+    def backward(ctx, *grads):
+        x, x2, feats, h0, hs, *ws = ctx.saved_tensors
+        (offs, P0, bound, cfg, step, has_x2, n_params, dims, half_mode, blob_density, blob_radius,
+         epsilon) = ctx.meta
+        none = (None,) * 18
+        if all(g is None for g in grads):
+            return none
+        P_active = _active_points(offs.shape[0], grads)
+        param = getattr(ctx, "param_ref", None)
+        with L.on(x):
+            dh0, dhs = _head_backward_train(h0, hs, x, x2 if has_x2 else None, offs, bound, blob_density, blob_radius,
+                                            epsilon, grads, P_active)
+            dplanes, wg = _backward_mlp_compact(dh0, dhs, feats, ws, dims, x, cfg, half_mode, P_active,
+                                                in_place=grid_ops.INPLACE_GRAD_PLANES and P_active == offs.shape[0]
+                                                and _last_pass_through_graph())
+            del dh0, dhs
+            gp = _park_or_scatter(param, ctx.forward_key, dplanes, x, x2 if has_x2 else None, offs, P0, bound, cfg, step,
+                                  n_params, P_active)
+        return (gp, *wg, *none[:11])
+
+
+def field_train(params, layers, x, offsets, cfg, bound, blob_density, blob_radius, x2=None, P0=None, step=0.0,
+                half_mode=None, epsilon=grid_ops.EPS):
+    P = np.asarray(offsets).reshape(-1, 3).shape[0]
+    if P0 is None:
+        P0 = P
+    out = _FieldTrain.apply(params, *mlp_ops.layer_args(layers), x, x2, offsets, P0, bound, cfg, step,
+                            _half_mode(half_mode), blob_density, blob_radius, epsilon)
+    return out if len(out) == 4 else (*out, None)
 
 
 @torch.no_grad()
diff --git a/make-it-3d_amd/mi3d/network.py b/make-it-3d_amd/mi3d/network.py
--- a/make-it-3d_amd/mi3d/network.py
+++ b/make-it-3d_amd/mi3d/network.py
@@ -138,8 +138,9 @@
         x = x.reshape(-1, 3).float()
         offs, P0 = grid_ops.stencil_offsets(center=True, second=x2 is not None)
         if x.is_cuda and self.sigma_net.fused_ok(x) and self.encoder.cfg["n_levels"] * 2 == self.sigma_net.dim_in:
-            return field_ops.field(self.encoder.params, self.sigma_net.net, x, offs, self.encoder.cfg, float(self.bound),
-                                   self.opt.blob_density, self.opt.blob_radius, x2, P0 if x2 is not None else None, step)
+            node = field_ops.field_train if self.training and x2 is not None else field_ops.field
+            return node(self.encoder.params, self.sigma_net.net, x, offs, self.encoder.cfg, float(self.bound),
+                        self.opt.blob_density, self.opt.blob_radius, x2, P0 if x2 is not None else None, step)
         sig, h = self._stencil_sigma(x, offs, x2, P0 if x2 is not None else None, step)
         albedo = self._sigmoid(h[:, 0, 1:])
         normals = self._normal_from(sig[:, 1:7])
```

Measured after the change: 11.08, median of 6. Within noise of the previous version (+1.2%).
